# LinjianMa/pairwise-perturbation

Hardware: AMD Instinct MI355X
Metric: ALS sweeps/sec (exact dimension-tree sweep, CP order-4 s=200 R=10) (higher is better)
Workload: dtype f32

## Files before the change

### include/ppals.h

```cpp
#ifndef PPALS_H
#define PPALS_H
#include <stdint.h>
#ifdef __cplusplus
extern "C" {
#endif

#define PPALS_F32 0
#define PPALS_F64 1

#define PPALS_OK 0
#define PPALS_ERR_NO_DEVICE (-1)
#define PPALS_ERR_HIP (-2)
#define PPALS_ERR_ARG (-3)
#define PPALS_ERR_COMM (-4)
#define PPALS_ERR_UNSUPPORTED (-5)
#define PPALS_MAX_ORDER 8
#define PPALS_UNIQUE_ID_BYTES 128

typedef struct ppals_ctx ppals_ctx;
typedef struct ppals_tensor ppals_tensor;
typedef struct ppals_cp ppals_cp;
typedef struct ppals_tucker ppals_tucker;

const char *ppals_last_error(void);
const char *ppals_version(void);

int ppals_preload_eigensolver(void);

int ppals_ctx_create(ppals_ctx **out, int device);
void ppals_ctx_destroy(ppals_ctx *ctx);
int ppals_get_unique_id(void *out128);
int ppals_ctx_init_comm(ppals_ctx *ctx, int rank, int nranks, const void *unique_id128);
int ppals_ctx_rank(const ppals_ctx *ctx);
int ppals_ctx_nranks(const ppals_ctx *ctx);
int ppals_ctx_sync(ppals_ctx *ctx);
int ppals_profile_enable(ppals_ctx *ctx, int level);
int ppals_profile_read(ppals_ctx *ctx, int which, int64_t *launches, double *total_ms,
                       double *algo_bytes);
int ppals_profile_reset(ppals_ctx *ctx);

int ppals_tensor_create(ppals_ctx *ctx, int order, const int64_t *global_lens, int dtype,
                        ppals_tensor **out);
void ppals_tensor_destroy(ppals_tensor *t);
int ppals_tensor_local_rows(const ppals_tensor *t, int64_t *lo, int64_t *n);
int ppals_tensor_fill_cp(ppals_tensor *t, int R, const double *Wtrue_flat);
int ppals_tensor_fill_uniform(ppals_tensor *t, uint64_t seed, double lo, double hi);
int ppals_tensor_fill_laplacian(ppals_tensor *t, int ndigits, int s);
int ppals_tensor_fill_collinear(ppals_tensor *t, int R, double col_min, double col_max,
                                double ratio_noise, uint64_t seed);
int ppals_collinear_factors(int order, const int64_t *lens, int R, double col_min, double col_max,
                            uint64_t seed, double *Wflat);
int ppals_tensor_upload(ppals_tensor *t, const double *host_full);
int ppals_tensor_download(ppals_tensor *t, double *host_full);

#define PPALS_F16 2
#define PPALS_BF16 3
int ppals_tensor_import_device(ppals_tensor *t, const void *src, int src_dtype, const int64_t *box_lo,
                               const int64_t *box_len, const int64_t *strides, void *stream);
int ppals_tensor_export_device(ppals_tensor *t, void *dst, int dst_dtype, const int64_t *box_lo,
                               const int64_t *box_len, const int64_t *strides, void *stream);
int ppals_tensor_check_device_view(ppals_tensor *t, int direction, const void *ptr, int dtype,
                                   const int64_t *box_lo, const int64_t *box_len,
                                   const int64_t *strides);
int ppals_tensor_norm(ppals_tensor *t, double *out);
void ppals_fill_uniform_host(double *out, int64_t n, uint64_t seed, uint64_t offset, double lo,
                             double hi);

int ppals_tree_node(ppals_cp *s, const char *key, double *out, int64_t *n);
int ppals_mttkrp(ppals_cp *s, int mode, double *M);
int ppals_pp_operator(ppals_cp *s, const char *contracted, double *out, int64_t *n);
int ppals_cp_residual(ppals_cp *s, double *out);
int ppals_cp_gram_system(ppals_cp *s, int mode, double lambda, double *S, double *Sinv);

int ppals_cp_create(ppals_ctx *ctx, ppals_tensor *V, int R, ppals_cp **out);
void ppals_cp_destroy(ppals_cp *s);
int ppals_cp_set_factors(ppals_cp *s, const double *Wflat, const double *gradWflat );
int ppals_cp_get_factors(ppals_cp *s, double *Wflat, double *gradWflat );
#define PPALS_SCHEDULE_DT 0
#define PPALS_SCHEDULE_MSDT 1
int ppals_cp_set_schedule(ppals_cp *s, int schedule);
int ppals_cp_get_schedule(const ppals_cp *s);
int ppals_cp_placement_report(const ppals_cp *s, char *buf, int cap);
int ppals_cp_pp_build_stats(ppals_cp *s, int mode, int64_t *builds, double *seconds);
int ppals_cp_sweeps_dt(ppals_cp *s, int n, double lambda);
int ppals_cp_gradnorm(ppals_cp *s, double *out);

typedef struct {
  double tol;
  double timelimit;
  int maxiter;
  double lambda;
  int resprint;
  int bench;
  double tol_init;
  double ratio_step;
  const char *csv_path;
  int csv_append;
  int verbose;
  double update_percentage;
} ppals_cp_opts;

int ppals_cp_dt(ppals_cp *s, const ppals_cp_opts *o, int *iters);
int ppals_cp_pp(ppals_cp *s, const ppals_cp_opts *o, int *iters);
int ppals_cp_pp_partupdate(ppals_cp *s, const ppals_cp_opts *o, int *iters);

#define PPALS_OPT_SIMPLE 0
#define PPALS_OPT_DT 1
#define PPALS_OPT_MSDT 2
int ppals_cpd_als(ppals_cp *s, int optimizer, const ppals_cp_opts *o, double *sweeps, int *iters);
#define PPALS_OPT_DT_LR 3
#define PPALS_OPT_MSDT_LR 4
int ppals_cpd_als_lr(ppals_cp *s, int optimizer, int update_rank, int randomsvd,
                     const ppals_cp_opts *o, double *sweeps, int *iters);

int ppals_tucker_create(ppals_ctx *ctx, ppals_tensor *V, const int *ranks, ppals_tucker **out);
void ppals_tucker_destroy(ppals_tucker *s);
int ppals_tucker_set_factors(ppals_tucker *s, const double *Wflat);
int ppals_tucker_set_core(ppals_tucker *s, const double *core);
int ppals_tucker_get_factors(ppals_tucker *s, double *Wflat, double *core);
int ppals_tucker_hosvd(ppals_tucker *s);
int ppals_tucker_ttmc(ppals_tucker *s, int skip, double *Y, int64_t *n);
int ppals_tucker_sweeps_dt(ppals_tucker *s, int n);
int ppals_tucker_dt(ppals_tucker *s, const ppals_cp_opts *o, int *iters);
int ppals_tucker_pp(ppals_tucker *s, const ppals_cp_opts *o, int *iters);

#define PPALS_MODEL 0
#define PPALS_RESIDUAL 1
int ppals_cp_export_model_device(ppals_cp *s, int what, void *dst, int dst_dtype, const int64_t *box_lo,
                                 const int64_t *box_len, const int64_t *strides, void *stream);
int ppals_tucker_export_model_device(ppals_tucker *s, int what, void *dst, int dst_dtype,
                                     const int64_t *box_lo, const int64_t *box_len,
                                     const int64_t *strides, void *stream);

#ifdef __cplusplus
}
#endif
#endif
```

### pairwise-perturbation_amd/csrc/engine.cpp

```cpp
#include "engine.h"
#include "run_report.h"

#include <algorithm>
#include <cmath>
#include <cstdio>
#include <cstdlib>
#include <cstring>
#include <fstream>
#include <iostream>
#include <stdexcept>

namespace ppals {

int tensor_create(Ops &ops, Comm &comm, int order, const int64_t *glens, int dtype,
                  TensorDesc *out, std::string *err) {
  if (order < 2 || order > MAX_ORDER) {
    *err = "tensor order must be in [2, 8]";
    return -1;
  }
  if (!ops.supports_storage(dtype))
    throw Unsupported(dtype == BF16 ? "ppals: this back end cannot store a bf16 tensor"
                                    : "ppals: this back end cannot store this tensor type");
  TensorDesc t;
  t.order = order;
// ... 132 lines not shown
        if (ok) break;
      }
    }
    W += s * R;
  }
  for (int i = 0; i < R; i++) {
    const double lambda_ = 0.2 + 0.6 / R * (i + 1);
    for (int64_t e = 0; e < lens[0]; e++) Wflat[e + lens[0] * i] *= lambda_;
  }
}

void tensor_fill_collinear(Ops &ops, Comm &comm, const TensorDesc &V, int R, double col_min,
                           double col_max, double ratio_noise, uint64_t seed) {
  size_t tot = 0;
  for (int i = 0; i < V.order; i++) tot += (size_t)V.glens[i] * R;
  std::vector<double> W(tot);
  collinear_factors(V.glens, V.order, R, col_min, col_max, seed, W.data());
  tensor_fill_cp(ops, V, R, W.data());
  const double vnorm = tensor_norm(ops, comm, V);
  double *d = (double *)ops.alloc(sizeof(double));
  const uint64_t nseed = seed + 0x5eedull;
  ops.uniform_sumsq(V.llens[0], V.glens[0], V.row0, rest_of(V), nseed, -1.0, 1.0, d);
  if (comm.size() > 1) comm.allreduce_sum(d, 1);
  double nsq = 0;
  ops.d2h(&nsq, d, sizeof(double));
  ops.free(d);
  const double alpha = ratio_noise * vnorm / std::sqrt(nsq);
  ops.add_uniform_noise(V.data, V.dtype, V.llens[0], V.glens[0], V.row0, rest_of(V), nseed, -1.0,
                        1.0, alpha);
  ops.sync();
}

double tensor_norm(Ops &ops, Comm &comm, const TensorDesc &V) {
  int64_t M, K;
  split_sizes(V, &M, &K);
  double *d = (double *)ops.alloc(sizeof(double));
  ops.residual_sq(V.data, V.dtype, M, K, nullptr, nullptr, 0, d);
  if (comm.size() > 1) comm.allreduce_sum(d, 1);
  double h = 0;
  ops.d2h(&h, d, sizeof(double));
  ops.free(d);
  return std::sqrt(h);
}

CpEngine::CpEngine(Ops &ops, Comm &comm, const TensorDesc &V, int R)
    : ops_(ops), comm_(comm), V_(V), N_(V.order), R_(R), P_(comm.size()), rank_(comm.rank()) {
  dist_ = P_ > 1 || (force_comm_path() && !comm.is_self());
  if (R <= 0) throw std::runtime_error("ppals: rank must be positive");
  residual_form_ = residual_form_env();
  W_.resize(N_);
  gradW_.resize(N_);
  Wprev_.assign(N_, nullptr);
  Winit_.assign(N_, nullptr);
  dW_.assign(N_, nullptr);
  dM_.assign(N_, nullptr);
  Mm_.assign(N_, nullptr);
  for (int i = 0; i < N_; i++) {
    size_t n = (size_t)V_.glens[i] * R_ * sizeof(double);
    W_[i] = (double *)ops_.alloc(n);
    gradW_[i] = (double *)ops_.alloc(n);
    ops_.zero(W_[i], n);
    ops_.zero(gradW_[i], n);
    maxs_ = std::max(maxs_, V_.glens[i]);
    maxblk_ = std::max(maxblk_, block_rows(V_.glens[i], P_));
  }
  G_ = (double *)ops_.alloc(sizeof(double) * N_ * R_ * R_);
  S_ = (double *)ops_.alloc(sizeof(double) * R_ * R_);
  Sinv_ = (double *)ops_.alloc(sizeof(double) * R_ * R_);
  gradsq_ = (double *)ops_.alloc(sizeof(double) * MAX_ORDER);
  scal_ = (double *)ops_.alloc(sizeof(double) * 4 * MAX_ORDER);
  ops_.zero(gradsq_, sizeof(double) * MAX_ORDER);
  if (dist_) {
    size_t n = sizeof(double) * (size_t)maxblk_ * P_ * R_;
    sendbuf_ = (double *)ops_.alloc(n);
    recvbuf_ = (double *)ops_.alloc(sizeof(double) * (size_t)maxblk_ * R_);
    gatherbuf_ = (double *)ops_.alloc(n);
    ops_.zero(sendbuf_, n);
    ops_.zero(gatherbuf_, n);
  }
  if (const char *e = std::getenv("PPALS_COMM_SMALL_BYTES")) small_msg_bytes_ = std::atoll(e);
  if (const char *e = std::getenv("PPALS_TEST_BLOCKED_UPDATE")) test_blocks_ = std::atoi(e);
  if (N_ < 3) schedule_ = 0;
  if (const char *e = std::getenv("PPALS_PLACE_TUNE")) ms_tune_enabled_ = std::atoi(e) != 0;
  if (N_ >= 3) {
    ms_set_roots(ms_choose_roots());
    ms_scales_ = (double *)ops_.alloc(sizeof(double) * 32);
  }
  if (V_.generation) tensor_gen_ = *V_.generation;
  {
    Layout nat;
    nat.ptr = V_.data;
    for (int m = 0; m < N_; m++) nat.order.push_back(m);
    lay_.push_back(nat);
  }
  size_t xmax = 0;
  const bool place = schedule_ == 1 && N_ >= 3 && ms_tune_enabled_ && ms_X_slack() > 0;
  if (place) {
    for (int r = 0; r < N_; r++) {
      if (ms_set_excluded(r, ms_k_, ms_excl_)) continue;
      xmax = std::max(xmax, ms_X_bytes(r, ms_k_));
    }
    const size_t avail = ops_.mem_available();
    const double tensor_bytes = (double)V_.nloc * dtype_size(V_.dtype);
    if (avail == (size_t)-1 || (double)avail > 2.0 * tensor_bytes + 6.0 * (double)(xmax + ms_X_slack()) + 8e9)
      ms_X_alt_ = ops_.try_alloc(xmax + ms_X_slack());
  }
  ensure_transposed();
  if (place) {
    ms_X_base_ = big_alloc(xmax + ms_X_slack());
    ms_X_cap_ = xmax + ms_X_slack();
  }
  for (int i = 0; i < MAX_ORDER; i++) grad_replicated_[i] = !dist_;
  build_tree(0, N_ - 1, -1);
  leaf_.assign(N_, -1);
  for (size_t k = 0; k < nodes_.size(); k++)
    if (nodes_[k].lo == nodes_[k].hi) leaf_[nodes_[k].lo] = (int)k;
}

void CpEngine::set_schedule(int schedule) {
  if (schedule != 0 && schedule != 1) throw std::runtime_error("ppals: unknown sweep schedule");
  schedule_ = (N_ < 3) ? 0 : schedule;
  for (auto &n : nodes_) n.valid = false;
  ms_invalidate();
}

CpEngine::~CpEngine() {
  try {
    ops_.sync();
  } catch (...) {
  }
  for (auto p : W_) ops_.free(p);
  for (auto p : gradW_) ops_.free(p);
  for (auto p : Wprev_) ops_.free(p);
  for (auto p : Winit_) ops_.free(p);
  for (auto p : dW_) ops_.free(p);
  for (auto p : dM_) ops_.free(p);
  for (auto p : Mm_) ops_.free(p);
  for (auto &n : nodes_) ops_.free(n.buf);
  lr_release();
  pp_clear();
  for (auto &kv : pp_pool_) ops_.free(kv.second.buf);
  ops_.free(pp_norms_);
  ops_.free(G_);
  ops_.free(S_);
  ops_.free(Sinv_);
  ops_.free(gradsq_);
  ops_.free(scal_);
  ops_.free(sendbuf_);
  ops_.free(recvbuf_);
  ops_.free(gatherbuf_);
  ops_.free(test_blkbuf_);
  ops_.free(Mbuf_);
  ops_.free(Qbuf_);
  ops_.free(xq_);
  ops_.free(xp_);
  ops_.free(Pbuf_);
  for (auto &l : lay_)
    if (l.owned) ops_.free(l.ptr);
  for (auto &ex : ms_place_)
    if (ex.timer >= 0) ops_.timer_read(ex.timer);
  ops_.free(ms_X_base_);
  ops_.free(ms_X_alt_);
  ops_.free(ms_scales_);
  for (auto &n : ms_nodes_) {
    ops_.free(n.t.buf);
    for (auto &t : n.tmp) ops_.free(t.buf);
// ... 44 lines not shown
        l.q = q;
        l.blk = b;
        l.ld = ld;
        return;
      }
    }
  };
  auto bytes_of = [&](const Layout &l) {
    return l.q ? (size_t)l.ld * (size_t)(V_.nloc / l.blk) * esz : (size_t)V_.nloc * esz;
  };
  const int mid = (N_ - 1) / 2;
  Layout t;
  for (int m = mid + 1; m < N_; m++) t.order.push_back(m);
  for (int m = 0; m <= mid; m++) t.order.push_back(m);
  choose_pad(t, std::min(N_ - 2, N_ - 1 - mid));
  int64_t min_ext = ext(0);
  for (int m = 1; m < N_; m++) min_ext = std::min(min_ext, ext(m));
  const size_t xbytes_max = (size_t)(V_.nloc / std::max<int64_t>(1, min_ext)) * R_ * esz;
  const size_t reserve = 3 * xbytes_max + ms_X_slack() + ((size_t)1 << 30);
  auto fits = [&](size_t bytes) {
    const size_t avail = ops_.mem_available();
    return avail == (size_t)-1 || avail >= bytes + reserve;
  };
  if (!fits(bytes_of(t))) return;
  t.ptr = ops_.try_alloc(bytes_of(t));
  if (!t.ptr) return;
  t.owned = true;
  t.bytes = bytes_of(t);
  fill_layout(t);
  lay_.push_back(t);
  vt_state_ = 1;
  Layout a;
  for (int m = 0; m < N_; m++) a.order.push_back(m);
  choose_pad(a, N_ - 2);
  if (a.q > 0 && fits(bytes_of(a))) {
    a.ptr = ops_.try_alloc(bytes_of(a));
    if (a.ptr) {
      a.owned = true;
      a.bytes = bytes_of(a);
      fill_layout(a);
      lay_.push_back(a);
    }
  }
}

bool CpEngine::plan_scan(int first, int k, bool natural_only, ScanPlan &plan) {
  auto in_set = [&](int m) { return ((m - first + N_) % N_) < k; };
  const int64_t line = 128 / (int64_t)dtype_size(V_.dtype);
  const Layout *best = nullptr;
  int best_p0 = 0;
  int64_t best_L = 0;
  bool best_al = false;
  const size_t nlay = natural_only ? 1 : lay_.size();
  for (size_t li = 0; li < nlay; li++) {
    const Layout &l = lay_[li];
    int p0 = -1;
    for (int p = 0; p < N_; p++)
      if (in_set(l.order[p])) {
        p0 = p;
        break;
      }
    int len = 0;
    while (p0 + len < N_ && in_set(l.order[p0 + len])) len++;
    if (len != k || (l.q > 0 && p0 < l.q)) continue;
    int64_t L = 1;
    for (int p = 0; p < p0; p++) L *= ext(l.order[p]);
    const bool al = L >= 256 && (l.q > 0 || L % line == 0);
    if (!best || (al && !best_al) ||
        (al == best_al && (L > best_L || (L == best_L && l.q > 0 && best->q == 0)))) {
      best = &l;
      best_p0 = p0;
      best_L = L;
      best_al = al;
    }
  }
  if (!best) return false;
  plan = ScanPlan();
  plan.lay = best;
  for (int p = 0; p < N_; p++) {
    const int m = best->order[p];
    if (p < best_p0) {
      plan.Lc *= ext(m);
      plan.kept.push_back(m);
    } else if (p < best_p0 + k) {
      plan.J *= ext(m);
      plan.set.push_back(m);
    } else {
      plan.T *= ext(m);
      plan.kept.push_back(m);
    }
  }
  plan.L = plan.Lc;
  if (best->q > 0) {
    plan.L = plan.Lc / best->blk * best->ld;
    plan.pad.ld = best->ld;
    plan.pad.valid = best->blk;
  }
  return true;
}

void CpEngine::check_tensor_generation() {
  if (!V_.generation || *V_.generation == tensor_gen_) return;
  tensor_gen_ = *V_.generation;
  for (const auto &l : lay_)
    if (l.owned) fill_layout(l);
  for (auto &n : nodes_) n.valid = false;
  ms_invalidate();
  pp_clear();
}

FactorRef CpEngine::fref(int m, double *const *W) const {
  FactorRef f;
  f.ptr = W[m] + (m == 0 ? V_.row0 : 0);
  f.rows = ext(m);
  f.ld = V_.glens[m];
  return f;
}
int64_t CpEngine::prod_ext(int lo, int hi) const {
  int64_t p = 1;
  for (int m = lo; m <= hi; m++) p *= ext(m);
  return p;
}

void CpEngine::build_tree(int lo, int hi, int parent) {
  if (hi <= lo) return;
  const int mid = (lo + hi) / 2;
  const int ranges[2][2] = {{lo, mid}, {mid + 1, hi}};
  int idx[2];
  for (int c = 0; c < 2; c++) {
    Node n;
    n.lo = ranges[c][0];
    n.hi = ranges[c][1];
    n.parent = parent;
    n.slo = ranges[1 - c][0];
    n.shi = ranges[1 - c][1];
    n.elems = 0;
    nodes_.push_back(n);
    idx[c] = (int)nodes_.size() - 1;
  }
  build_tree(lo, mid, idx[0]);
  build_tree(mid + 1, hi, idx[1]);
}
int CpEngine::find_node(int lo, int hi) const {
  for (size_t k = 0; k < nodes_.size(); k++)
    if (nodes_[k].lo == lo && nodes_[k].hi == hi) return (int)k;
  return -1;
}

void CpEngine::compute_node(int idx) {
  check_tensor_generation();
  Node &n = nodes_[idx];
  if (n.valid) return;
  n.elems = prod_ext(n.lo, n.hi);
  if (!n.buf) n.buf = (double *)ops_.alloc(sizeof(double) * (size_t)n.elems * R_);
  FactorRef f[MAX_ORDER];
  int nf = 0;
  for (int m = n.slo; m <= n.shi; m++) f[nf++] = fref(m, W_.data());
  const int64_t J = prod_ext(n.slo, n.shi);
  const bool sib_is_suffix = n.slo > n.hi;
  if (n.parent < 0) {
    ScanPlan pl;
    if (!plan_scan(n.slo, n.shi - n.slo + 1, false, pl))
      throw std::runtime_error("ppals: internal error (tree node not adjacent)");
    if (pl.Lc == 1 && !sib_is_suffix) {
      ops_.scan_contract(V_.data, V_.dtype, 1, J, n.elems, f, nf, R_, n.buf, F64, 1, n.elems);
    } else {
// ... 204 lines not shown
  }
}

bool CpEngine::ms_set_excluded(int first, int k, unsigned excl) const {
  for (int q = 0; q < k; q++)
    if ((excl >> ((first + q) % N_)) & 1u) return true;
  return false;
}

int CpEngine::ms_next_root(int i, int k, unsigned excl) const {
  int first = (i - k + N_) % N_, guard = 0;
  while (ms_set_excluded(first, k, excl) && guard++ < N_) first = (first - 1 + N_) % N_;
  if (ms_set_excluded(first, k, excl) || ((i - first + N_) % N_) < k) return -1;
  return first;
}

double CpEngine::ms_schedule_cost(int k, unsigned excl) const {
  int root = -1;
  double cost = 0;
  const int sweeps = 2 * N_;
  for (int u = 0; u < (sweeps + 2) * N_; u++) {
    const int i = u % N_;
    if (root < 0 || ((i - root + N_) % N_) < k) {
      root = ms_next_root(i, k, excl);
      if (root < 0) return 1e300;
      if (u >= 2 * N_) {
        double J = 1;
        for (int q = 0; q < k; q++) J *= (double)ext((root + q) % N_);
        cost += 1.0 + 4.5 * (double)R_ / J;
      }
    }
  }
  return cost / sweeps;
}

int CpEngine::ms_choose_roots() {
  const unsigned mandatory = (dist_ && N_ > 2) ? 1u : 0u;
  const int kcap = dist_ ? std::max(1, (N_ - 1) / 2) : N_;
  int kfix = 0;
  if (const char *e = std::getenv("PPALS_MSDT_ROOTS")) {
    const int k = std::atoi(e);
    if (k >= 1 && k <= N_ - 2) kfix = std::min(k, kcap);
  }
  unsigned small = 0;
  for (int m = 0; m < N_; m++)
    if ((double)R_ >= 0.05 * (double)ext(m)) small |= 1u << m;
  int best = 1;
  unsigned best_excl = mandatory;
  double best_cost = 1e300;
  for (int k = 1; k <= std::max(1, N_ / 2) && k <= N_ - 2 && k <= kcap; k++) {
    if (kfix && k != kfix) continue;
    for (unsigned sub = small;; sub = (sub - 1) & small) {
      const unsigned excl = sub | mandatory;
      const double cost = ms_schedule_cost(k, excl);
      const bool tie = cost <= best_cost * (1.0 + 1e-9) && cost >= best_cost * (1.0 - 1e-9);
      if (cost < best_cost * (1.0 - 1e-9) ||
          (tie && k == best && __builtin_popcount(excl) < __builtin_popcount(best_excl))) {
        best_cost = cost;
        best = k;
        best_excl = excl;
      }
      if (sub == 0) break;
    }
  }
  if (best_cost >= 1e299) {
    best = 1;
    best_excl = mandatory;
  }
  ms_excl_ = best_excl;
  return best;
}

void CpEngine::ms_set_roots(int k) {
  for (auto &n : ms_nodes_) {
    ops_.free(n.t.buf);
    for (auto &t : n.tmp) ops_.free(t.buf);
  }
  ms_nodes_.clear();
  ms_k_ = k;
  ms_build_tree(0, N_ - k - 1, -1);
  ms_leaf_.assign(N_ - k, -1);
  for (size_t q = 0; q < ms_nodes_.size(); q++)
    if (ms_nodes_[q].lo == ms_nodes_[q].hi) ms_leaf_[ms_nodes_[q].lo] = (int)q;
  if (ms_nodes_.size() + 1 > 32) throw std::runtime_error("ppals: tensor order too large");
  ms_X_.slot = 0;
  for (size_t q = 0; q < ms_nodes_.size(); q++) ms_nodes_[q].t.slot = (int)q + 1;
  ms_invalidate();
}

double CpEngine::place_min_bytes() {
  const char *e = std::getenv("PPALS_PLACE_MIN_MB");
  return e ? std::atof(e) * 1048576.0 : 1.5e9;
}

size_t CpEngine::ms_X_slack() const {
  const double bytes = (double)V_.nloc * dtype_size(V_.dtype);
  return bytes >= place_min_bytes() ? ((size_t)64 << 20) + 4096 : 0;
}

void CpEngine::ms_place_collect(PlaceExplore &ex) {
  if (ex.timer < 0) return;
  const double t = ops_.timer_read(ex.timer);
  ex.timer = -1;
  if (t <= 0 || ex.timer_cand < 0 || ex.timer_cand >= (int)ex.cands.size()) return;
  PlaceCand &c = ex.cands[ex.timer_cand];
  c.best = std::min(c.best, t);
  c.samples++;
  ex.worst = std::max(ex.worst, t);
}

int CpEngine::ms_place_pick(PlaceExplore &ex) {
  ms_place_collect(ex);
  if (ex.phase == 0) {
    int n = 0, best0 = -1;
    double lo = 1e300, hi = 0;
    for (size_t q = 0; q < ex.cands.size(); q++)
      if (ex.cands[q].samples > 0) {
        n++;
        lo = std::min(lo, ex.cands[q].best);
        hi = std::max(hi, ex.cands[q].best);
        if (ex.cands[q].blk == 0 && (best0 < 0 || ex.cands[q].best < ex.cands[best0].best)) best0 = (int)q;
      }
    if (n >= kPlaceGateSamples && best0 >= 0 && hi < lo * (1.0 + kPlaceGateSpread)) {
      ex.chosen = best0;
      ex.gated = true;
      ex.phase = 2;
      ms_place_release_unchosen();
      return -1;
    }
  }
  if (ex.phase == 0 && ex.next >= ex.cands.size()) {
    std::vector<int> idx(ex.cands.size());
    for (size_t q = 0; q < idx.size(); q++) idx[q] = (int)q;
    std::stable_sort(idx.begin(), idx.end(),
                     [&](int a, int b) { return ex.cands[a].best < ex.cands[b].best; });
    const size_t nfin = std::min<size_t>(3, idx.size());
    for (size_t q = 0; q < nfin; q++)
      for (int kind = 0; kind < 2; kind++) {
        PlaceCand c;
        c.blk = ex.cands[idx[q]].blk;
        c.off = ex.cands[idx[q]].off;
        c.nt = kind;
        ex.cands.push_back(c);
      }
    ex.phase = 1;
  }
  if (ex.phase == 1 && ex.next >= ex.cands.size()) {
    int best = -1;
    for (size_t q = 0; q < ex.cands.size(); q++)
      if (ex.cands[q].samples > 0 && (best < 0 || ex.cands[q].best < ex.cands[best].best * 0.995))
        best = (int)q;
    ex.chosen = best;
    ex.phase = 2;
    ms_place_release_unchosen();
  }
  return ex.phase < 2 ? (int)ex.next++ : -1;
}

void CpEngine::ms_place_release_unchosen() {
  if (!ms_X_alt_) return;
  bool use[2] = {false, false};
  for (const auto &ex : ms_place_) {
    if (ex.phase == 0 || ex.phase == 1) return;
    if (ex.phase == 2) use[ex.chosen >= 0 ? ex.cands[ex.chosen].blk : 0] = true;
  }
  if (use[0] && use[1]) return;
  ops_.sync();
  if (!use[1]) {
    ops_.free(ms_X_alt_);
  } else {
    ops_.free(ms_X_base_);
    ms_X_base_ = ms_X_alt_;
    for (auto &ex : ms_place_)
      for (auto &c : ex.cands) c.blk = 0;
  }
  ms_X_alt_ = nullptr;
}

size_t CpEngine::ms_X_bytes(int first, int k) const {
  int64_t J = 1;
  for (int q = 0; q < k; q++) J *= ext((first + q) % N_);
  return (size_t)(V_.nloc / J) * R_ * dtype_size(work_dt(V_.dtype));
}

void *CpEngine::big_alloc(size_t bytes) {
  for (;;) {
    void *p = ops_.try_alloc(bytes);
    if (p) return p;
    if (ms_X_alt_ && !(ms_X_.valid && (char *)ms_X_.buf >= (char *)ms_X_alt_ &&
                       (char *)ms_X_.buf < (char *)ms_X_alt_ + ms_X_cap_)) {
      ops_.sync();
      for (auto &ex : ms_place_) {
        if (ex.timer >= 0) {
          ops_.timer_read(ex.timer);
          ex.timer = -1;
        }
        for (auto &c : ex.cands) c.blk = 0;
      }
      ops_.free(ms_X_alt_);
      ms_X_alt_ = nullptr;
      continue;
    }
    if (lay_.size() > 1 && lay_.back().owned) {
      ops_.sync();
      ops_.free(lay_.back().ptr);
      lay_.pop_back();
      if (lay_.size() == 1) vt_state_ = -1;
      for (auto &n : nodes_) n.valid = false;
      continue;
    }
    return ops_.alloc(bytes);
  }
}

void CpEngine::ms_start_step(int first) {
  const int k = ms_k_;
  ms_root_ = first;
  ms_order_.clear();
  for (int q = k; q < N_; q++) ms_order_.push_back((first + q) % N_);
  for (auto &n : ms_nodes_) n.t.valid = false;
  const size_t xbytes = ms_X_bytes(first, k);
  const size_t slack = ms_tune_enabled_ ? ms_X_slack() : 0;
  if (!ms_X_override_ && ms_X_cap_ < xbytes + slack) {
    for (auto &ex : ms_place_) {
      if (ex.timer >= 0) ops_.timer_read(ex.timer);
      ex = PlaceExplore();
    }
    ops_.free(ms_X_base_);
    ops_.free(ms_X_alt_);
    ms_X_base_ = ms_X_alt_ = nullptr;
    ms_X_cap_ = 0;
    ms_X_base_ = big_alloc(xbytes + slack);
    ms_X_cap_ = xbytes + slack;
  }
  ScanPlan pl;
  if (!plan_scan(first, k, false, pl)) {
    if (k == 1) throw std::runtime_error("ppals: internal error (single root not adjacent)");
    ms_set_roots(1);
    int r = (first + k - 1) % N_, guard = 0;
    while (((ms_excl_ >> r) & 1u) && guard++ < N_) r = (r - 1 + N_) % N_;
    ms_start_step(r);
    return;
  }
  const void *src = pl.lay->ptr;
  const int64_t L = pl.Lc, J = pl.J, T = pl.T;
  ms_X_.modes = pl.kept;
  std::vector<FactorRef> f;
  unsigned mask = 0;
  for (int m : pl.set) {
    f.push_back(fref(m, W_.data()));
    mask |= 1u << m;
  }
  ms_X_.dt = work_dt(V_.dtype);
  ms_X_.contracted = mask;
  if ((size_t)L * T * R_ * dtype_size(ms_X_.dt) != xbytes)
    throw std::runtime_error("ppals: internal error (first-level intermediate size)");
  auto launch_scan = [&](int blk, int64_t off, int nt) {
    ms_X_.buf = ms_X_override_ ? (char *)ms_X_override_
                               : (char *)(blk == 1 && ms_X_alt_ ? ms_X_alt_ : ms_X_base_) + off;
    ops_.scan_store_mode(nt);
    ops_.scan_contract(src, V_.dtype, pl.L, J, T, f.data(), (int)f.size(), R_, ms_X_.buf, ms_X_.dt,
                       L, L * T, pl.pad);
    ops_.scan_store_mode(-1);
  };
  PlaceExplore &ex = ms_place_[first];
  if (slack > 0 && !ms_X_override_ && ex.phase < 0) {
    static const int64_t cand_small[] = {0, 1, 2, 3, 4, 5, 6, 8, 12, 16, 24, 32, 48, 64};
    static const int64_t cand_large[] = {0, 3, 5, 12, 16, 24, 48, 64};
    const double bytes = (double)L * J * T * dtype_size(V_.dtype);
    ex.phase = 3;
    ex.layout = (int)(pl.lay - lay_.data());
    if (bytes >= place_min_bytes() && R_ <= 32 && (double)xbytes >= 0.01 * bytes) {
      const bool large = bytes >= 2e10;
      const int64_t *mb = large ? cand_large : cand_small;
      for (int ci = 0; ci < (large ? 8 : 14); ci++) {
        if ((size_t)(mb[ci] << 20) > slack) break;
        PlaceCand c;
        c.off = mb[ci] << 20;
        ex.cands.push_back(c);
      }
      static const int64_t cand_alt[] = {0, 4, 16, 64};
      for (int ci = 0; ms_X_alt_ && ci < 4; ci++) {
        if ((size_t)(cand_alt[ci] << 20) > slack) break;
        PlaceCand c;
        c.blk = 1;
        c.off = cand_alt[ci] << 20;
        ex.cands.push_back(c);
      }
      ex.phase = 0;
    }
  }
  const int cand = (slack > 0 && !ms_X_override_ && ex.phase >= 0 && ex.phase < 2) ? ms_place_pick(ex) : -1;
  if (cand >= 0) {
    ex.visits++;
    ex.timer_cand = cand;
    ex.timer = ops_.timer_begin();
    launch_scan(ex.cands[cand].blk, ex.cands[cand].off, ex.cands[cand].nt);
    if (ex.timer >= 0) ops_.timer_end(ex.timer);
  } else if (ex.phase == 2 && ex.chosen >= 0 && slack > 0 && !ms_X_override_) {
    launch_scan(ex.cands[ex.chosen].blk, ex.cands[ex.chosen].off, ex.cands[ex.chosen].nt);
  } else {
    launch_scan(0, 0, -1);
  }
  ms_X_.pending = false;
  ms_X_.valid = true;
  if (const char *tr = std::getenv("PPALS_TRACE_STEPS")) {
    if (FILE *f = std::fopen(tr, "a")) {
      const int li = (int)(pl.lay - lay_.data());
      std::fprintf(f, "rank=%d root=%d k=%d layout=%s%s L=%lld J=%lld T=%lld\n", rank_, first, k,
                   li == 1 ? "VT" : "V", pl.lay->q > 0 ? "pad" : "", (long long)L, (long long)J,
                   (long long)T);
      std::fclose(f);
    }
  }
}

void CpEngine::ms_mode_update(int i, double lambda, bool last_of_sweep) {
  check_tensor_generation();
  if (ms_root_ < 0 || ((i - ms_root_ + N_) % N_) < ms_k_) {
    const int first = ms_next_root(i, ms_k_, ms_excl_);
    if (first < 0) throw std::runtime_error("ppals: no root set without the excluded modes");
    ms_start_step(first);
  }
  int pos = -1;
  for (size_t q = 0; q < ms_order_.size(); q++)
    if (ms_order_[q] == i) pos = (int)q;
  const int leaf = ms_leaf_[pos];
  ops_.arm_gram_system(G_, N_, i, R_, lambda, S_, Sinv_);
  ms_compute(leaf);
  ms_norm_fused_ = false;
  if (last_of_sweep && (!dist_ || (i != 0 && (int64_t)sizeof(double) * V_.glens[i] * R_ <= small_msg_bytes_))) {
    int64_t rows[MAX_ORDER];
    for (int q = 0; q < N_; q++) rows[q] = V_.glens[q];
    if (ops_.arm_normalize(W_.data(), rows, N_, R_, G_, i, nullptr)) {
      unsigned masks[32] = {0}, fresh = 0;
      const unsigned active = ms_collect_scales(masks, &fresh, leaf);
      ms_norm_fused_ = ops_.arm_normalize(W_.data(), rows, N_, R_, G_, i, nullptr, ms_scales_, masks, active, fresh);
    }
  }
  mode_update(i, (const double *)ms_nodes_[leaf].t.buf, ext(i), lambda, false, 1.0);
  ms_nodes_[leaf].t.valid = false;
}

void CpEngine::ms_contract(const RTensor &src, int mode, RTensor &dst, const double *in_scale) {
  int64_t L = 1, T = 1;
  bool before = true;
  dst.modes.clear();
  for (int m : src.modes) {
    if (m == mode) {
      before = false;
      continue;
    }
    (before ? L : T) *= ext(m);
    dst.modes.push_back(m);
  }
  dst.dt = F64;
  dst.contracted = src.contracted | (1u << mode);
  ms_reserve(dst, sizeof(double) * (size_t)L * T * R_);
  FactorRef f = fref(mode, W_.data());
  ops_.mttv(src.buf, src.dt, L, ext(mode), T, &f, 1, R_, (double *)dst.buf, L * T, 0, in_scale);
}

void CpEngine::ms_compute(int idx) {
  MsNode &n = ms_nodes_[idx];
  if (n.t.valid) return;
  const RTensor *src;
  if (n.parent < 0) {
    src = &ms_X_;
  } else {
    ms_compute(n.parent);
    src = &ms_nodes_[n.parent].t;
  }
  std::vector<int> sib;
  for (int pos = n.slo; pos <= n.shi; pos++) sib.push_back(ms_order_[pos]);
  auto storage_pos = [&](int mode) {
    for (size_t k = 0; k < src->modes.size(); k++)
      if (src->modes[k] == mode) return (int)k;
    return -1;
  };
  std::sort(sib.begin(), sib.end(), [&](int a, int b) { return storage_pos(a) > storage_pos(b); });
  if (n.tmp.size() + 1 < sib.size()) n.tmp.resize(sib.size() - 1);
  const RTensor *cur = src;
  for (size_t k = 0; k < sib.size(); k++) {
    RTensor &dst = (k + 1 == sib.size()) ? n.t : n.tmp[k];
    ms_contract(*cur, sib[k], dst, k == 0 ? ms_scale_of(*src) : nullptr);
    cur = &dst;
  }
  if (sib.empty()) throw std::runtime_error("ppals: empty sibling set in the multi-sweep tree");
  n.t.pending = false;
  n.t.valid = true;
}

void CpEngine::sweep_msdt(double lambda) {
  for (int i = 0; i < N_; i++) ms_mode_update(i, lambda, i == N_ - 1);
  if (!ms_norm_fused_) normalize();
  ms_norm_fused_ = false;
  grad_from_sweep_ = true;
}

void CpEngine::sweep_dt(double lambda) {
  if (schedule_ == 1) {
    sweep_msdt(lambda);
    return;
  }
  for (auto &n : nodes_) n.valid = false;
  bool norm_fused = false;
  for (int i = 0; i < N_; i++) {
    compute_node(leaf_[i]);
    const Node &lf = nodes_[leaf_[i]];
    if (i == N_ - 1 && !dist_) {
      int64_t rows[MAX_ORDER];
      for (int q = 0; q < N_; q++) rows[q] = V_.glens[q];
      norm_fused = ops_.arm_normalize(W_.data(), rows, N_, R_, G_, i, nullptr);
    }
    mode_update(i, lf.buf, ext(i), lambda, false, 1.0);
  }
  if (!norm_fused) normalize();
  grad_from_sweep_ = true;
}

void CpEngine::update_modes(int first, int count, double lambda) {
  for (int k = 0; k < count; k++) {
    const int i = (first + k) % N_;
    if (schedule_ == 1) {
      ms_mode_update(i, lambda);
    } else {
      if (i == 0 || k == 0)
        for (auto &n : nodes_) n.valid = false;
      compute_node(leaf_[i]);
      mode_update(i, nodes_[leaf_[i]].buf, ext(i), lambda, false, 1.0);
    }
  }
  grad_from_sweep_ = true;
}

void CpEngine::lr_release() {
  for (int m = 0; m < MAX_ORDER; m++) {
    ops_.free(lr_cache_[m]);
    lr_cache_[m] = nullptr;
    lr_have_[m] = false;
  }
  ops_.free(lr_X_);
  ops_.free(lr_Us_);
  ops_.free(lr_G2_);
  ops_.free(lr_small_);
  ops_.free(lr_T_);
  lr_X_ = lr_Us_ = lr_G2_ = lr_small_ = lr_T_ = nullptr;
  lr_T_cap_ = 0;
}

void CpEngine::lr_step_begin(int left, bool reuse, int r) {
  check_tensor_generation();
  if (ms_k_ != 1) ms_set_roots(1);
  if (!lr_cache_[left]) lr_cache_[left] = big_alloc(ms_X_bytes(left, 1));
  if (reuse && lr_have_[left]) {
    ScanPlan pl;
    if (!plan_scan(left, 1, false, pl)) throw std::runtime_error("ppals: internal error (LR scan plan)");
    const int64_t n = pl.Lc * pl.T;
    if (lr_T_cap_ < sizeof(double) * (size_t)n * r) {
      ops_.free(lr_T_);
      lr_T_ = (double *)ops_.alloc(sizeof(double) * (size_t)n * r);
      lr_T_cap_ = sizeof(double) * (size_t)n * r;
    }
    FactorRef f;
    f.ptr = lr_Us_ + (left == 0 ? V_.row0 : 0);
    f.rows = ext(left);
    f.ld = V_.glens[left];
    ops_.scan_contract(pl.lay->ptr, V_.dtype, pl.L, ext(left), pl.T, &f, 1, r, lr_T_, F64, pl.Lc, n,
                       pl.pad);
    ops_.lowrank_accumulate(lr_cache_[left], work_dt(V_.dtype), n, R_, lr_T_, r, lr_small_);
    ms_X_ = lr_desc_[left];
    ms_X_.buf = lr_cache_[left];
    ms_X_.valid = true;
    ms_X_.pending = false;
    ms_root_ = left;
    ms_order_.clear();
    for (int q = 1; q < N_; q++) ms_order_.push_back((left + q) % N_);
    for (auto &nd : ms_nodes_) nd.t.valid = false;
  } else {
    ms_X_override_ = lr_cache_[left];
    ms_start_step(left);
    ms_X_override_ = nullptr;
    lr_desc_[left] = ms_X_;
    lr_have_[left] = true;
  }
}

static void host_qr_mgs2(int n, int k, double *A) {
  for (int j = 0; j < k; j++) {
    double *aj = A + (size_t)n * j;
    for (int pass = 0; pass < 2; pass++)
      for (int p = 0; p < j; p++) {
        const double *ap = A + (size_t)n * p;
        double d = 0;
        for (int i = 0; i < n; i++) d += ap[i] * aj[i];
        for (int i = 0; i < n; i++) aj[i] -= d * ap[i];
      }
    double nn = 0;
    for (int i = 0; i < n; i++) nn += aj[i] * aj[i];
    nn = std::sqrt(nn);
    for (int i = 0; i < n; i++) aj[i] = nn > 0 ? aj[i] / nn : 0.0;
  }
}
static void host_jacobi_eig(int n, double *A, double *ev, double *V) {
  for (int i = 0; i < n; i++)
    for (int j = 0; j < n; j++) V[i + (size_t)n * j] = i == j ? 1.0 : 0.0;
  for (int sweep = 0; sweep < 60; sweep++) {
    double off = 0, diag = 0;
    for (int i = 0; i < n; i++)
      for (int j = 0; j < n; j++) (i == j ? diag : off) += A[i + (size_t)n * j] * A[i + (size_t)n * j];
    if (off <= 1e-30 * (diag + 1e-300)) break;
    for (int p = 0; p < n - 1; p++)
      for (int q = p + 1; q < n; q++) {
        const double apq = A[p + (size_t)n * q];
        if (apq == 0.0) continue;
        const double theta = (A[q + (size_t)n * q] - A[p + (size_t)n * p]) / (2.0 * apq);
        const double t = (theta >= 0 ? 1.0 : -1.0) / (std::fabs(theta) + std::sqrt(theta * theta + 1.0));
        const double c = 1.0 / std::sqrt(t * t + 1.0), sn = t * c;
        for (int k = 0; k < n; k++) {
          const double akp = A[k + (size_t)n * p], akq = A[k + (size_t)n * q];
          A[k + (size_t)n * p] = c * akp - sn * akq;
          A[k + (size_t)n * q] = sn * akp + c * akq;
        }
        for (int k = 0; k < n; k++) {
          const double apk = A[p + (size_t)n * k], aqk = A[q + (size_t)n * k];
          A[p + (size_t)n * k] = c * apk - sn * aqk;
          A[q + (size_t)n * k] = sn * apk + c * aqk;
        }
        for (int k = 0; k < n; k++) {
          const double vkp = V[k + (size_t)n * p], vkq = V[k + (size_t)n * q];
          V[k + (size_t)n * p] = c * vkp - sn * vkq;
          V[k + (size_t)n * q] = sn * vkp + c * vkq;
        }
      }
  }
  std::vector<int> idx(n);
  for (int i = 0; i < n; i++) idx[i] = i;
  std::sort(idx.begin(), idx.end(), [&](int a, int b) { return A[a + (size_t)n * a] > A[b + (size_t)n * b]; });
  std::vector<double> Vs((size_t)n * n);
  for (int k = 0; k < n; k++) {
    ev[k] = A[idx[k] + (size_t)n * idx[k]];
    for (int i = 0; i < n; i++) Vs[i + (size_t)n * k] = V[i + (size_t)n * idx[k]];
  }
  std::copy(Vs.begin(), Vs.end(), V);
}
static const uint64_t LR_RANDOM_SEED = 0x52414e44535644ull;

void CpEngine::lr_mode_update(int i, double lambda, int r, const double *base) {
  int pos = -1;
  for (size_t q = 0; q < ms_order_.size(); q++)
    if (ms_order_[q] == i) pos = (int)q;
  if (pos < 0) throw std::runtime_error("ppals: internal error (LR update of the root mode)");
  const int leaf = ms_leaf_[pos];
  ms_compute(leaf);
  const double *M = (const double *)ms_nodes_[leaf].t.buf;
  const int64_t s = V_.glens[i];
  if (r <= 0) {
    mode_update(i, M, ext(i), lambda, false, 1.0);
    ms_nodes_[leaf].t.valid = false;
    return;
  }
// ... 871 lines not shown
```

### pairwise-perturbation_amd/csrc/engine.h

```cpp
#pragma once
#include <cstdint>
#include <cstdlib>
#include <map>
#include <string>
#include <vector>

#include "ops.h"

namespace ppals {

struct TensorDesc {
  int order = 0;
  int64_t glens[MAX_ORDER];
  int64_t llens[MAX_ORDER];
  int64_t row0 = 0;
  int dtype = F32;
  void *data = nullptr;
  int64_t nloc = 0;
  const uint64_t *generation = nullptr;
};

inline int64_t block_rows(int64_t s, int P) { return (s + P - 1) / P; }
inline bool force_comm_path() {
  const char *v = getenv("PPALS_FORCE_COMM");
  return v && atoi(v) != 0;
}

enum ResidualForm { RESIDUAL_FUSED = 0, RESIDUAL_TWO_PASS = 1 };
int residual_form_env();
struct ModelExportCall {
  const ViewArgs *a;
  const TensorDesc *V;
  void *dst;
  bool residual;
  int form;
  bool exported = false;
  void *stream;
};
void model_export_run(Ops &ops, ModelExportCall &c, const ModelPlan &mp, const double *Q, const double *P,
                      int K);

int tensor_create(Ops &ops, Comm &comm, int order, const int64_t *glens, int dtype,
                  TensorDesc *out, std::string *err);
void tensor_fill_cp(Ops &ops, const TensorDesc &V, int R, const double *Wtrue_flat);
void tensor_fill_uniform(Ops &ops, const TensorDesc &V, uint64_t seed, double lo, double hi);
void tensor_upload(Ops &ops, const TensorDesc &V, const double *host_full);
void tensor_download(Ops &ops, const TensorDesc &V, double *host_full);
void tensor_fill_laplacian(Ops &ops, const TensorDesc &V, int ndigits, int s);
void collinear_factors(const int64_t *lens, int N, int R, double col_min, double col_max,
                       uint64_t seed, double *Wflat);
void tensor_fill_collinear(Ops &ops, Comm &comm, const TensorDesc &V, int R, double col_min,
                           double col_max, double ratio_noise, uint64_t seed);
double tensor_norm(Ops &ops, Comm &comm, const TensorDesc &V);

struct CpOpts {
  double tol = 0, timelimit = 5e3;
  int maxiter = 0;
  double lambda = 0;
  int resprint = 10;
  int bench = 0;
  double tol_init = 1e-2, ratio_step = 1.0;
  double update_percentage = 1.0;
  int update_rank = 0;
  int randomsvd = 0;
  std::string csv_path;
  bool csv_append = false;
  bool verbose = false;
};

class RunReport;
struct ModeNorms;

class CpEngine {
 public:
  CpEngine(Ops &ops, Comm &comm, const TensorDesc &V, int R);
  ~CpEngine();

  void set_factors(const double *Wflat, const double *gradWflat);
  void set_schedule(int schedule);
  int schedule() const { return schedule_; }
  std::string placement_report() const;
  void pp_build_stats(int mode, int64_t *builds, double *seconds) {
    if (builds) *builds = pp_builds_;
    if (seconds) *seconds = pp_build_s_;
    if (mode != 0) {
      pp_builds_ = 0;
      pp_build_s_ = 0;
      pp_build_timed_ = mode > 0;
    }
  }
  void get_factors(double *Wflat, double *gradWflat);

  void sweep_dt(double lambda);
  double gradnorm();
  double residual();
  void export_model(const ViewArgs &a, void *dst, bool residual, void *stream);
  const TensorDesc &tensor() const { return V_; }

  int64_t tree_node(const std::string &key, double *out_host);
  void mttkrp(int mode, double *M_host);
  int64_t pp_operator(const std::string &contracted, double *out_host);
  void gram_system(int mode, double lambda, double *S_host, double *Sinv_host);

  int run_dt(const CpOpts &o, int *iters);
  int run_pp(const CpOpts &o, int *iters);
  int run_pp_partupdate(const CpOpts &o, int *iters);
  int run_class(int kind, const CpOpts &o, double *sweeps, int *iters);
  void update_modes(int first, int count, double lambda);


  int order() const { return N_; }
  int rank_r() const { return R_; }

 private:
  struct Node {
    int lo, hi;
    int parent = -1;
    int slo, shi;
    double *buf = nullptr;
    int64_t elems = 0;
    bool valid = false;
  };
  struct PPOp {
    void *buf = nullptr;
    int dt = F64;
    int64_t elems = 0;
    std::vector<int> modes;
    bool owned = true;
    const double *scale = nullptr;
  };
  struct PPBuf {
    void *buf = nullptr;
    size_t cap = 0;
  };
  std::map<std::string, PPBuf> pp_pool_;
  void *pp_buffer(const std::string &seq, size_t bytes);
  bool pp_norms_live_ = false;
  double *pp_norms_ = nullptr;

  struct RTensor {
    void *buf = nullptr;
    size_t cap = 0;
    int dt = F64;
    std::vector<int> modes;
    unsigned contracted = 0;
    int slot = -1;
    bool pending = false;
    bool valid = false;
  };
  struct MsNode {
    int lo, hi, parent, slo, shi;
    RTensor t;
    std::vector<RTensor> tmp;
  };
  void ms_build_tree(int lo, int hi, int parent);
  void ms_start_step(int root);
  void ms_compute(int idx);
  void ms_reserve(RTensor &t, size_t bytes);
  void ms_contract(const RTensor &src, int mode, RTensor &dst, const double *in_scale);
  void sweep_msdt(double lambda);
  void ms_invalidate() { ms_root_ = -1; }
  int schedule_ = 1;
  int ms_root_ = -1;
  int ms_k_ = 1;
  int test_blocks_ = 0;
  double *test_blkbuf_ = nullptr;
  unsigned ms_excl_ = 0;
  bool ms_set_excluded(int first, int k, unsigned excl) const;
  int ms_next_root(int i, int k, unsigned excl) const;
  double ms_schedule_cost(int k, unsigned excl) const;
  int ms_choose_roots();
  void ms_set_roots(int k);
  void ms_mode_update(int i, double lambda, bool last_of_sweep = false);
  bool ms_norm_fused_ = false;
  unsigned ms_collect_scales(unsigned *masks, unsigned *fresh, int skip_node);
  RTensor ms_X_;
  struct PlaceCand {
    int blk = 0;
    int64_t off = 0;
    int nt = -1;
    double best = 1e300;
    int samples = 0;
  };
  struct PlaceExplore {
    int phase = -1;
    size_t next = 0;
    int timer = -1;
    int timer_cand = -1;
    int chosen = -1;
    int layout = 0;
    double worst = 0;
    int visits = 0;
    bool gated = false;
    std::vector<PlaceCand> cands;
  };
  static constexpr int kPlaceGateSamples = 8;
  static constexpr double kPlaceGateSpread = 0.04;
  PlaceExplore ms_place_[MAX_ORDER];
  void ms_place_collect(PlaceExplore &ex);
  int ms_place_pick(PlaceExplore &ex);
  void *ms_X_base_ = nullptr;
  void *ms_X_alt_ = nullptr;
  void ms_place_release_unchosen();
  size_t ms_X_cap_ = 0;
  int64_t pp_builds_ = 0;
  double pp_build_s_ = 0;
  bool pp_build_timed_ = false;
  bool ms_tune_enabled_ = true;
  size_t ms_X_slack() const;
  static double place_min_bytes();
  size_t ms_X_bytes(int first, int k) const;
  void *big_alloc(size_t bytes);
  std::vector<MsNode> ms_nodes_;
  void lr_step_begin(int left, bool reuse, int r);
  void lr_mode_update(int i, double lambda, int r, const double *base);
  void lr_release();
  void *lr_cache_[MAX_ORDER] = {nullptr};
  bool lr_have_[MAX_ORDER] = {false};
  bool lr_random_ = false;
  uint64_t lr_random_calls_ = 0;
  RTensor lr_desc_[MAX_ORDER];
  void *ms_X_override_ = nullptr;
  double *lr_X_ = nullptr, *lr_Us_ = nullptr, *lr_G2_ = nullptr, *lr_small_ = nullptr;
  double *lr_T_ = nullptr;
  size_t lr_T_cap_ = 0;


  std::vector<int> ms_order_;
  std::vector<int> ms_leaf_;
  double *ms_scales_ = nullptr;
  const double *ms_scale_of(const RTensor &t) const { return t.pending ? ms_scales_ + t.slot : nullptr; }

  int64_t ext(int m) const { return m == 0 ? V_.llens[0] : V_.glens[m]; }
  FactorRef fref(int m, double *const *W) const;
  int64_t prod_ext(int lo, int hi) const;
  void build_tree(int lo, int hi, int parent);
  int find_node(int lo, int hi) const;
  void compute_node(int idx);
  void refresh_grams();
  void mode_update(int i, const double *M, int64_t ldm, double lambda, bool pp, double ratio);
  void normalize();
  const PPOp &pp_get(const std::string &seq);
  int pp_last_mode(const std::string &seq) const;
  std::string pp_parent(const std::string &seq) const;
  void pp_contract_pair(const PPOp &T, int cmode, const FactorRef &f, double *out, int64_t out_rows);
  bool pp_fast_ = true;
  bool pp_no_borrow_ = false;
  void pp_clear();
  void pp_build_all();
  void sweep_pp(double lambda, double ratio);
  double allreduce_scalar(double x);
  bool agree(bool local);
  ModeNorms read_norms(bool dt_phase);
  bool print_block(RunReport &rep, const CpOpts &o, int iter, int pp_flag, double &projnorm,
                   bool bench);
  void dt_sub(RunReport &rep, const CpOpts &o, double &projnorm, int &iter);
  void pp_restart();
  void pp_sub(RunReport &rep, const CpOpts &o, double &projnorm, int &iter);
  void pp_partupdate_sub(RunReport &rep, const CpOpts &o, double &projnorm, int &iter);
  int run_pp_common(const CpOpts &o, int *iters, bool partupdate);

  Ops &ops_;
  Comm &comm_;
  TensorDesc V_;
  int N_, R_, P_, rank_;
  bool dist_ = false;
  std::vector<double *> W_, gradW_, Wprev_, Winit_, dW_, dM_, Mm_;
  double *G_ = nullptr;
  double *S_ = nullptr, *Sinv_ = nullptr;
  double *gradsq_ = nullptr;
  double *scal_ = nullptr;
  double *sendbuf_ = nullptr, *recvbuf_ = nullptr, *gatherbuf_ = nullptr;
  double *Mbuf_ = nullptr;
  double *Qbuf_ = nullptr, *Pbuf_ = nullptr;
  double *xq_ = nullptr, *xp_ = nullptr;
  int64_t xq_cap_ = 0, xp_cap_ = 0;
  int residual_form_ = RESIDUAL_FUSED;
  struct Layout {
    void *ptr = nullptr;
    std::vector<int> order;
    int q = 0;
    int64_t blk = 0, ld = 0;
    bool owned = false;
    size_t bytes = 0;
  };
  std::vector<Layout> lay_;
  int vt_state_ = 0;
  uint64_t tensor_gen_ = 0;
  void ensure_transposed();
  void fill_layout(const Layout &l);
  struct ScanPlan {
    const Layout *lay = nullptr;
    int64_t L = 1, Lc = 1, J = 1, T = 1;
    RowPad pad;
    std::vector<int> set, kept;
  };
  bool plan_scan(int first, int k, bool natural_only, ScanPlan &plan);
  void check_tensor_generation();
  int64_t small_msg_bytes_ = 1 << 20;
  bool grad_replicated_[MAX_ORDER];
  int64_t maxs_ = 0, maxblk_ = 0;
  std::vector<Node> nodes_;
  std::vector<int> leaf_;
  std::map<std::string, PPOp> pp_;
  bool grad_from_sweep_ = false;
  double init_gradnorm_ = 0;
};

}
```

### pairwise-perturbation_amd/csrc/hip_ops.hip

```cpp
#include <dlfcn.h>
#include <hip/hip_runtime.h>
#include <chrono>

#include <algorithm>
#include <cstdio>
#include <cstdlib>
#include <stdexcept>
#include <string>
#include <map>
#include <type_traits>
#include <vector>

#include "hip_ops.h"
#include "roctx_ranges.h"
#include "preload_policy.h"
#include "kernels_scan.hip.h"
#include "kernels_small.hip.h"
#include "kernels_eig.hip.h"
#include "kernels_io.hip.h"
#include "kernels_model.hip.h"
#include "kernels_bf16.hip.h"

namespace ppals {
#define HIP_CHECK(expr)                                                                       \
// ... 28 lines not shown

template <auto V, auto... Vs, typename T, typename F>
static inline void dispatch(T v, F &&f) {
  if constexpr (sizeof...(Vs) == 0)
    f(std::integral_constant<decltype(V), V>());
  else if (v == V)
    f(std::integral_constant<decltype(V), V>());
  else
    dispatch<Vs...>(v, f);
}

struct EigLibs {
  void *blas = nullptr, *solver = nullptr;
};
static bool g_hip_runtime_up = false;
static EigLibs &eig_libs() {
  static EigLibs l;
  if (l.blas && l.solver) return l;
  switch (late_preload_policy(false, g_hip_runtime_up, getenv("PPALS_STRICT_PRELOAD"))) {
    case kPreloadRefuse: throw Unsupported(late_preload_message());
    case kPreloadWarn: fprintf(stderr, "%s\n", late_preload_message()); fflush(stderr); break;
    default: break;
  }
  l.blas = dlopen("librocblas.so.5", RTLD_NOW | RTLD_GLOBAL);
  if (!l.blas) l.blas = dlopen("librocblas.so", RTLD_NOW | RTLD_GLOBAL);
  l.solver = dlopen("librocsolver.so.0", RTLD_NOW | RTLD_GLOBAL);
  if (!l.solver) l.solver = dlopen("librocsolver.so", RTLD_NOW | RTLD_GLOBAL);
  if (!l.blas || !l.solver)
    throw std::runtime_error(std::string("ppals: cannot load rocSOLVER: ") + dlerror());
  return l;
}

class HipOps : public Ops {
 public:
  explicit HipOps(int device) {
    int ndev = 0;
    hipError_t e = hipGetDeviceCount(&ndev);
    if (e != hipSuccess || ndev <= 0)
      throw std::runtime_error(
          "ppals: no HIP device available (the engine has no CPU fallback; hipGetDeviceCount: " +
          std::string(e == hipSuccess ? "0 devices" : hipGetErrorString(e)) + ")");
    if (device < 0 || device >= ndev)
      throw std::runtime_error("ppals: device index out of range");
    dev_ = device;
    g_hip_runtime_up = true;
    HIP_CHECK(hipSetDevice(dev_));
    HIP_CHECK(hipStreamCreateWithFlags(&st_, hipStreamNonBlocking));
    hipDeviceProp_t prop;
    HIP_CHECK(hipGetDeviceProperties(&prop, dev_));
    ncu_ = prop.multiProcessorCount;
    HIP_CHECK(hipFuncSetAttribute((const void *)k_gram_system,
                                  hipFuncAttributeMaxDynamicSharedMemorySize, 96 * 1024));
    HIP_CHECK(hipFuncSetAttribute((const void *)k_cp_update,
                                  hipFuncAttributeMaxDynamicSharedMemorySize, 96 * 1024));
    HIP_CHECK(hipFuncSetAttribute((const void *)k_top_eig_small,
                                  hipFuncAttributeMaxDynamicSharedMemorySize, 152 * 1024));
    HIP_CHECK(hipFuncSetAttribute((const void *)k_cp_mode_update<false, false>,
                                  hipFuncAttributeMaxDynamicSharedMemorySize, 152 * 1024));
    HIP_CHECK(hipFuncSetAttribute((const void *)k_cp_mode_update<true, true>,
                                  hipFuncAttributeMaxDynamicSharedMemorySize, 152 * 1024));
    if (const char *v = getenv("PPALS_FORCE_JACOBI")) force_jacobi_ = atoi(v);
    if (const char *v = getenv("PPALS_EIG_FAST")) {
      eig_fast_ = atoi(v);
      eig_cold_ = eig_fast_ != 2;
    }
    if (const char *v = getenv("PPALS_EIG_DEBUG")) eig_debug_ = atoi(v);
    if (const char *v = getenv("PPALS_EIG_SIGMA_SCALE")) eig_sigma_scale_ = atof(v);
    if (const char *v = getenv("PPALS_FORCE_EIGINV")) force_eiginv_ = atoi(v);
    HIP_CHECK(hipFuncSetAttribute((const void *)k_chol_rinv,
                                  hipFuncAttributeMaxDynamicSharedMemorySize, 72 * 1024));
    HIP_CHECK(hipFuncSetAttribute((const void *)k_chol_m,
                                  hipFuncAttributeMaxDynamicSharedMemorySize, 152 * 1024));
    HIP_CHECK(hipFuncSetAttribute((const void *)k_rr_apply,
                                  hipFuncAttributeMaxDynamicSharedMemorySize, 152 * 1024));
    if (const char *v = getenv("PPALS_SYM_LDS_MIN")) sym_lds_min_ = std::max(32, atoi(v));
    if (const char *v = getenv("PPALS_EIG_DEFER")) {
      eig_defer_ok_ = atoi(v);
      handover_ok_ = eig_defer_ok_ != 2;
    }
    if (const char *v = getenv("PPALS_EIG_DEFER_FAIL")) eig_defer_fail_ = atoi(v);
    if (const char *v = getenv("PPALS_SCAN_TAIL")) scan_tail_on_ = atoi(v) != 0;
    if (const char *v = getenv("PPALS_SCAN_WIDE")) wide_enabled_ = atoi(v) != 0;
    if (const char *v = getenv("PPALS_COLD_SUBSPACE_FROM")) cold_subspace_from_ = std::max(65, atoi(v));
    if (const char *v = getenv("PPALS_PERSIST_MULT")) persist_mult_ = std::max(1, atoi(v));
    HIP_CHECK(hipFuncSetAttribute((const void *)k_rmult_chol,
                                  hipFuncAttributeMaxDynamicSharedMemorySize, 152 * 1024));
    HIP_CHECK(hipFuncSetAttribute((const void *)k_jacobi_onesided,
                                  hipFuncAttributeMaxDynamicSharedMemorySize, 152 * 1024));
    HIP_CHECK(hipFuncSetAttribute((const void *)k_rr_small,
                                  hipFuncAttributeMaxDynamicSharedMemorySize, 152 * 1024));
    HIP_CHECK(hipFuncSetAttribute((const void *)k_gram_system_lds,
                                  hipFuncAttributeMaxDynamicSharedMemorySize, 152 * 1024));
    HIP_CHECK(hipFuncSetAttribute((const void *)k_gram_system_mfma,
                                  hipFuncAttributeMaxDynamicSharedMemorySize, 152 * 1024));
    if (const char *v = getenv("PPALS_GJ_SCALAR")) gj_scalar_ = atoi(v);
  }
  ~HipOps() override {
    hipSetDevice(dev_);
    hipStreamSynchronize(st_);
    if (st2_) hipStreamSynchronize(st2_);
    for (auto &ev : events_) {
      hipEventDestroy(ev.a);
      hipEventDestroy(ev.b);
    }
    for (auto &t : timers_) {
      hipEventDestroy(t.a);
      hipEventDestroy(t.b);
    }
    if (ws_mttv_) hipFree(ws_mttv_);
    if (ws_pack_) hipFree(ws_pack_);
    if (ws_mv_) hipFree(ws_mv_);
    if (ws_slab_) hipFree(ws_slab_);
    if (ws_krp_) hipFree(ws_krp_);
    if (ws_part_) hipFree(ws_part_);
    if (ws_small_) hipFree(ws_small_);
    if (ws_big_) hipFree(ws_big_);
    if (ws_big2_) hipFree(ws_big2_);
    if (ws_eig_) hipFree(ws_eig_);
    if (ws_orth_) hipFree(ws_orth_);
    if (ws_pow_) hipFree(ws_pow_);
    if (ws_cold_) hipFree(ws_cold_);
    if (ws_cold2_) hipFree(ws_cold2_);
    if (ws_cholm_) hipFree(ws_cholm_);
    if (ws_gsfb_) hipFree(ws_gsfb_);
    if (ws_jac_) hipFree(ws_jac_);
    if (eig_host_) hipHostFree(eig_host_);
    if (ws_part2_) hipFree(ws_part2_);
    for (auto &kv : eig_state_) {
      if (kv.second.Q) hipFree(kv.second.Q);
      if (kv.second.Qn) hipFree(kv.second.Qn);
      free_lazy(kv.second);
    }
    for (auto &kv : eig_small_)
      if (kv.second.Q) hipFree(kv.second.Q);
    if (st2_) hipStreamDestroy(st2_);
    if (handover_) hipFree(handover_);
    if (io_ev_in_) hipEventDestroy(io_ev_in_);
    if (io_ev_out_) hipEventDestroy(io_ev_out_);
    hipStreamDestroy(st_);
  }

  void *alloc(size_t bytes) override {
    void *p = nullptr;
    HIP_CHECK(hipSetDevice(dev_));
    HIP_CHECK(hipMalloc(&p, bytes ? bytes : 8));
    return p;
  }
  void free(void *p) override {
    if (p) {
      hipStreamSynchronize(st_);
      hipFree(p);
    }
  }
  void h2d(void *dst, const void *src, size_t bytes) override {
    HIP_CHECK(hipMemcpyAsync(dst, src, bytes, hipMemcpyHostToDevice, st_));
    HIP_CHECK(hipStreamSynchronize(st_));
  }
  void d2h(void *dst, const void *src, size_t bytes) override {
    HIP_CHECK(hipMemcpyAsync(dst, src, bytes, hipMemcpyDeviceToHost, st_));
    HIP_CHECK(hipStreamSynchronize(st_));
  }
  void d2d(void *dst, const void *src, size_t bytes) override {
    HIP_CHECK(hipMemcpyAsync(dst, src, bytes, hipMemcpyDeviceToDevice, st_));
  }
  void zero(void *p, size_t bytes) override { HIP_CHECK(hipMemsetAsync(p, 0, bytes, st_)); }
  void sync() override { HIP_CHECK(hipStreamSynchronize(st_)); }
  void *stream() override { return (void *)st_; }
  void bind() override { HIP_CHECK(hipSetDevice(dev_)); }
  bool supports_storage(int dt) override { return dt == F32 || dt == F64 || dt == BF16; }

  void fill_uniform(void *V, int dt, int64_t l0, int64_t g0, int64_t row0, int64_t rest,
                    uint64_t seed, double lo, double hi) override {
    int64_t n = l0 * rest;
    int g = grid_for(n, 256, 16384);
    if (dt == F32)
      hipLaunchKernelGGL(k_fill_uniform<float>, dim3(g), dim3(256), 0, st_, (float *)V, l0, g0,
                         row0, rest, seed, lo, hi);
    else if (dt == BF16)
      hipLaunchKernelGGL(k_fill_uniform<bf16s>, dim3(g), dim3(256), 0, st_, (bf16s *)V, l0, g0,
                         row0, rest, seed, lo, hi);
    else
      hipLaunchKernelGGL(k_fill_uniform<double>, dim3(g), dim3(256), 0, st_, (double *)V, l0, g0,
                         row0, rest, seed, lo, hi);
    HIP_CHECK(hipGetLastError());
  }

  void fill_laplacian(void *V, int dt, int64_t l0, int64_t g0, int64_t row0, int64_t rest,
                      int ndigits, int s) override {
    int g = grid_for(l0 * rest, 256, 16384);
    if (dt == F32)
      hipLaunchKernelGGL(k_fill_laplacian<float>, dim3(g), dim3(256), 0, st_, (float *)V, l0, g0,
                         row0, rest, ndigits, s);
    else if (dt == BF16)
      hipLaunchKernelGGL(k_fill_laplacian<bf16s>, dim3(g), dim3(256), 0, st_, (bf16s *)V, l0, g0,
                         row0, rest, ndigits, s);
// ... 413 lines not shown
  }

  void *try_alloc(size_t bytes) override {
    void *p = nullptr;
    hipSetDevice(dev_);
    if (hipMalloc(&p, bytes ? bytes : 8) != hipSuccess) {
      (void)hipGetLastError();
      return nullptr;
    }
    return p;
  }
  void scan_store_mode(int mode) override { scan_nt_mode_ = mode; }
  int scan_nt_mode_ = -1;
  size_t mem_available() override {
    size_t fr = 0, tot = 0;
    hipSetDevice(dev_);
    if (hipMemGetInfo(&fr, &tot) != hipSuccess) {
      (void)hipGetLastError();
      return (size_t)-1;
    }
    return fr;
  }
  void unpack_shards(const void *stage, int dt, int64_t s0, int64_t rest, int64_t blk, int P,
                     int64_t chunk_bytes, void *full) override {
    const int g = grid_for(s0 * rest, 256, 16384);
    if (dt == F32)
      hipLaunchKernelGGL(k_unpack_shards<float>, dim3(g), dim3(256), 0, st_, (const char *)stage,
                         s0, rest, blk, P, chunk_bytes, (float *)full);
    else if (dt == BF16)
      hipLaunchKernelGGL(k_unpack_shards<bf16s>, dim3(g), dim3(256), 0, st_, (const char *)stage,
                         s0, rest, blk, P, chunk_bytes, (bf16s *)full);
    else
      hipLaunchKernelGGL(k_unpack_shards<double>, dim3(g), dim3(256), 0, st_, (const char *)stage,
                         s0, rest, blk, P, chunk_bytes, (double *)full);
    HIP_CHECK(hipGetLastError());
  }
  void transpose2d(const void *src, int dt, int64_t rows, int64_t cols, void *dst) override {
    transpose_batched(src, dt, rows, cols, 1, dst);
  }
  void transpose_batched(const void *src, int dt, int64_t rows, int64_t cols, int64_t batch,
                         void *dst) override {
    const int64_t nb = ((rows + 63) / 64) * ((cols + 63) / 64);
    if (nb > 0x7fffffff) throw std::runtime_error("ppals: transpose grid too large");
    const size_t step = (size_t)rows * cols * dtype_size(dt);
    for (int64_t b0 = 0; b0 < batch; b0 += 65535) {
      const unsigned nby = (unsigned)std::min<int64_t>(65535, batch - b0);
      const char *s = (const char *)src + b0 * step;
      char *d = (char *)dst + b0 * step;
      if (dt == F32)
        hipLaunchKernelGGL(k_transpose<float>, dim3((unsigned)nb, nby), dim3(256), 0, st_,
                           (const float *)s, rows, cols, (float *)d);
      else if (dt == BF16)
        hipLaunchKernelGGL(k_transpose<bf16s>, dim3((unsigned)nb, nby), dim3(256), 0, st_,
                           (const bf16s *)s, rows, cols, (bf16s *)d);
      else
        hipLaunchKernelGGL(k_transpose<double>, dim3((unsigned)nb, nby), dim3(256), 0, st_,
                           (const double *)s, rows, cols, (double *)d);
    }
    HIP_CHECK(hipGetLastError());
  }

  static KrpArgs krp_args(const FactorRef *f, int nf, int64_t *J) {
    KrpArgs a;
    int64_t j = 1;
    if (nf > MAX_ORDER) throw std::runtime_error("ppals: too many Khatri-Rao factors");
    for (int i = 0; i < nf; i++) {
      a.ptr[i] = f[i].ptr;
      a.rows[i] = f[i].rows;
      a.ld[i] = f[i].ld;
      j *= f[i].rows;
    }
    a.nf = nf;
    *J = j;
    return a;
  }
  void krp(double *out, const FactorRef *f, int nf, int col0, int ncols) override {
    int64_t J;
    KrpArgs a = krp_args(f, nf, &J);
    hipLaunchKernelGGL(k_krp, dim3(grid_for(J * ncols, 256)), dim3(256), 0, st_, out, a, J, col0,
                       ncols);
    HIP_CHECK(hipGetLastError());
  }

  template <typename TV>
  void scan_t(const TV *V, int64_t L, int64_t J, int64_t T, const FactorRef *f, int nf, int R,
              double *out, int64_t out_tstride, int64_t out_rstride, int out32, RowPad pad) {
    constexpr int VEC = ScanTraits<TV>::VEC;
    int64_t Jc;
    KrpArgs a = krp_args(f, nf, &Jc);
    if (Jc != J) throw std::runtime_error("ppals: scan_contract factor extents do not match J");
    if (pad.ld && (L % pad.ld || pad.ld % VEC || pad.valid > pad.ld || pad.valid <= 0 || L == 1))
      throw std::runtime_error("ppals: scan_contract padded rows inconsistent");
    const bool aligned_base = (((uintptr_t)V) & 15) == 0;
    const bool wide_ok = sizeof(TV) == 4 && wide_enabled_ && L > 1 && aligned_base && (L % 4 == 0) &&
                         L >= 4 && (double)L * J * T >= 1.0e6 && 16.0 * (double)L * 4.0 < 2.0e9 &&
                         ((double)J / 16.0 + 1.0) * 8.0 * 1024.0 < 2.0e9;
    int col_step = 64;
    for (int col0 = 0; col0 < R; col0 += col_step) {
      if (wide_ok && R - col0 > 64) {
        col_step = std::min(128, R - col0);
        if constexpr (sizeof(TV) == 4)
          scan_wide((const float *)V, L, J, T, a, col0, col_step, out, out_tstride, out_rstride, out32, pad);
        continue;
      }
      col_step = 64;
      const int ncols = std::min(64, R - col0);
      const int NT = ncols <= 16 ? 1 : (ncols <= 32 ? 2 : (ncols <= 48 ? 3 : 4));
      const int64_t nblk64 = (J + 4 * VEC - 1) / (4 * VEC);
      if (nblk64 > 0x7fffffff) throw std::runtime_error("ppals: contraction extent too large");
      const int nblk = (int)nblk64;
      const size_t pack_bytes = (size_t)nblk * NT * 4 * 16 * VEC * sizeof(TV);
      TV *P = (TV *)ensure(ws_pack_, ws_pack_sz_, pack_bytes);
      const bool prefix = (L == 1);
      hipLaunchKernelGGL(k_krp_pack<TV>, dim3(grid_for((int64_t)nblk * NT * 64 * VEC, 256)),
                         dim3(256), 0, st_, P, nblk, NT, prefix ? 1 : 0, a, J, col0, ncols);
      HIP_CHECK(hipGetLastError());
      double *o = out32 ? (double *)((float *)out + (int64_t)col0 * out_rstride)
                        : out + (int64_t)col0 * out_rstride;
      const double bytes = (double)L * (double)J * (double)T * sizeof(TV) +
                           (double)L * (double)T * ncols * (out32 ? 4.0 : 8.0);
      if (prefix) {
        const int64_t M = J, K = T;
        const bool al = aligned_base && (M % VEC == 0);
        const int64_t ncolgrp = (K + 63) / 64;
        int want = 1;
        const int target = ncu_ * 4;
        if (ncolgrp < target) want = (int)std::min<int64_t>((target + ncolgrp - 1) / ncolgrp,
                                                            std::max(1, nblk / 64));
        const KSplit ks = k_split(nblk, want);
        const int nsplit = ks.nsplit, per = (int)ks.per;
        double *dst = o;
        int dst32 = out32;
        int64_t dst_ks = out_tstride, dst_ns = out_rstride, dst_ss = 0;
        if (nsplit > 1) {
          dst32 = 0;
          dst = (double *)ensure(ws_slab_, ws_slab_sz_, sizeof(double) * nsplit * ncols * K);
          dst_ks = 1;
          dst_ns = K;
          dst_ss = (int64_t)ncols * K;
        }
        dim3 grid((unsigned)ncolgrp, (unsigned)nsplit);
        dim3 grid_il((unsigned)((K + 15) / 16), (unsigned)nsplit);
        prof_begin(0, bytes);
        dispatch<1, 2, 3, 4>(NT, [&](auto nt) {
          if (al && M >= VEC)
            hipLaunchKernelGGL((k_scan_prefix_fast<TV, nt, 12>), grid_il, dim3(256), 0, st_, V, M, K, P, per,
                               nblk, dst, dst_ks, dst_ns, dst_ss, ncols, dst32);
          else
            dispatch<true, false>(al, [&](auto alv) {
              hipLaunchKernelGGL((k_scan_prefix<TV, nt, alv, 4>), grid, dim3(256), 0, st_, V, M, K, P, per,
                                 nblk, dst, dst_ks, dst_ns, dst_ss, ncols, dst32);
            });
        });
        prof_end();
        HIP_CHECK(hipGetLastError());
        slab_combine(nsplit, dst, dst_ss, K, ncols, o, out_tstride, out_rstride, out32);
      } else {
        const int64_t M = L, K = J;
        const bool al = aligned_base && (M % VEC == 0);
        const int64_t n_mtiles64 = (M + 64 * VEC - 1) / (64 * VEC);
        const int n_mtiles = (int)n_mtiles64;
        int want = 1;
        const int target = ncu_ * 8;
        if (T == 1 && n_mtiles < target)
          want = (int)std::min<int64_t>((target + n_mtiles - 1) / n_mtiles,
                                        std::max(1, nblk / 32));
        else if (T > 1 && n_mtiles64 * T < ncu_ && (double)M * T * ncols * nblk / 4 * 8.0 < 64e6)
          want = (int)std::min<int64_t>(((int64_t)ncu_ * 2 + n_mtiles64 * T - 1) / (n_mtiles64 * T),
                                        std::max(1, nblk / 4));
        const KSplit ks = k_split(nblk, want);
        const int nsplit = ks.nsplit, per = (int)ks.per;
        const PassDst d = pass_dst(nsplit, M, T, ncols, o, out32, out_rstride, out_tstride, pad);
        const int64_t nblocks = (int64_t)n_mtiles * nsplit * T;
        if (nblocks > 0x7fffffff) throw std::runtime_error("ppals: scan grid too large");
        dim3 grid((unsigned)nblocks);
        prof_begin(0, bytes);
        const int64_t pgrid = nblocks < (int64_t)ncu_ * persist_mult_ ? (int64_t)ncu_ * std::min(persist_mult_, 6)
                                                                       : (int64_t)ncu_ * persist_mult_;
        dim3 grid_p((unsigned)std::min<int64_t>(nblocks, pgrid));
        bool nts = nt_store(nsplit, (double)M * T * ncols * (d.out32 ? 4.0 : 8.0));
        const bool buf_ok = (16.0 * (double)M * sizeof(TV) < 2.0e9) && (pack_bytes < 2000000000ull);
        const bool takes_buf = al && M >= VEC && buf_ok && (NT == 1 || sizeof(TV) == 8) &&
                               !(sizeof(TV) == 8 && nsplit > 1);
        const bool takes_tail = !takes_buf && al && M >= VEC && T == 1 && nsplit == 1 && NT <= 2 &&
                                d.row_ld == 0 && scan_tail_split<TV>(NT, n_mtiles) >= 0;
        if (takes_tail) nts = false;
        if (takes_tail) {
          const int tail_from = scan_tail_split<TV>(NT, n_mtiles);
          const int64_t strips = ((M + 16 * VEC - 1) / (16 * VEC)) - (int64_t)tail_from * 4;
          dim3 grid_t((unsigned)(tail_from + strips));
          const size_t lds_t = sizeof(double) * 3 * (size_t)(VEC * NT * 4) * 64;
          dispatch<1, 2>(NT, [&](auto nt) {
            hipLaunchKernelGGL((k_scan_suffix_fast<TV, nt, 9>), grid_t, dim3(256), lds_t, st_, V, M, K, M * K, P,
                               n_mtiles, nsplit, per, nblk, d.p, d.nstride, d.split_stride, d.batch_stride, ncols,
                               d.out32, (int64_t)0, (int64_t)0, tail_from);
          });
        } else {
          dispatch<1, 2, 3, 4>(NT, [&](auto nt) {
            if (takes_buf)
              dispatch<5, 1>(nts ? 5 : 1, [&](auto opt) {
                hipLaunchKernelGGL((k_scan_suffix_buf<TV, nt, opt>), grid_p, dim3(256), 0, st_, V, M, K, M * K, P,
                                   n_mtiles, nsplit, per, nblk, d.p, d.nstride, d.split_stride, d.batch_stride,
                                   ncols, d.out32, nblocks, d.row_ld, d.row_valid);
              });
            else if (al && M >= VEC)
              dispatch<5, 1>(nts ? 5 : 1, [&](auto opt) {
                hipLaunchKernelGGL((k_scan_suffix_fast<TV, nt, opt>), grid, dim3(256), 0, st_, V, M, K, M * K, P,
                                   n_mtiles, nsplit, per, nblk, d.p, d.nstride, d.split_stride, d.batch_stride,
                                   ncols, d.out32, d.row_ld, d.row_valid);
              });
            else
              dispatch<true, false>(al, [&](auto alv) {
                hipLaunchKernelGGL((k_scan_suffix<TV, nt, alv>), grid, dim3(256), 0, st_, V, M, K, M * K, P,
                                   n_mtiles, nsplit, per, nblk, d.p, d.nstride, d.split_stride, d.batch_stride,
                                   ncols, d.out32, d.row_ld, d.row_valid);
              });
          });
        }
        prof_end();
        HIP_CHECK(hipGetLastError());
        slab_combine(nsplit, d.p, d.split_stride, M, ncols, o, 1, out_rstride, out32, pad, T, d.batch_stride,
                     out_tstride);
      }
    }
  }
  void scan_wide(const float *V, int64_t L, int64_t J, int64_t T, const KrpArgs &a, int col0, int ncols,
                 double *out, int64_t out_tstride, int64_t out_rstride, int out32, RowPad pad) {
    const int NT = (ncols + 15) / 16;
    const int64_t nblk64 = (J + 15) / 16;
    if (nblk64 > 0x7fffffff) throw std::runtime_error("ppals: contraction extent too large");
    const int nblk = (int)nblk64;
    const size_t pack_bytes = (size_t)nblk * NT * 256 * sizeof(float);
    float *P = (float *)ensure(ws_pack_, ws_pack_sz_, pack_bytes);
    hipLaunchKernelGGL(k_krp_pack<float>, dim3(grid_for((int64_t)nblk * NT * 256, 256)), dim3(256), 0, st_,
                       P, nblk, NT, 0, a, J, col0, ncols);
    HIP_CHECK(hipGetLastError());
    double *o = out32 ? (double *)((float *)out + (int64_t)col0 * out_rstride)
                      : out + (int64_t)col0 * out_rstride;
    const int64_t M = L, K = J;
    const int64_t n_mtiles64 = (M + 63) / 64;
    if (n_mtiles64 * T > 0x7fffffff) throw std::runtime_error("ppals: scan grid too large");
    const int n_mtiles = (int)n_mtiles64;
    const void *kernel = nullptr;
    dispatch<5, 6, 7, 8>(NT, [&](auto nt) { kernel = (const void *)k_scan_wide<nt, 1>; });
    const double slots = (double)ncu_ * occupancy(wide_occ_[NT - 1], kernel, 512, 0, 2);
    const int64_t tiles = n_mtiles64 * T;
    int want = 1;
    if ((double)tiles < 8.0 * slots) {
      double best = -1.0;
      const int ns_max = (int)std::min<int64_t>(24, std::max(1, nblk / 16));
      for (int ns = 1; ns <= ns_max; ns++) {
        const double rounds = (double)tiles * ns / slots;
        const double score = rounds / std::ceil(rounds) - 0.004 * ns;
        if (score > best) {
          best = score;
          want = ns;
        }
      }
    }
    const KSplit ks = k_split(nblk, want);
    const int nsplit = ks.nsplit, per = (int)ks.per;
    const PassDst d = pass_dst(nsplit, M, T, ncols, o, out32, out_rstride, out_tstride, pad);
    const int64_t nblocks = (int64_t)n_mtiles * nsplit * T;
    if (nblocks > 0x7fffffff) throw std::runtime_error("ppals: scan grid too large");
    const double bytes = (double)L * (double)J * (double)T * 4.0 + (double)L * (double)T * ncols * (out32 ? 4.0 : 8.0);
    prof_begin(0, bytes);
    dispatch<5, 6, 7, 8>(NT, [&](auto nt) {
      hipLaunchKernelGGL((k_scan_wide<nt, 1>), dim3((unsigned)nblocks), dim3(512), 0, st_, V, M, K, M * K, P,
                         n_mtiles, nsplit, per, nblk, d.p, d.nstride, d.split_stride, d.batch_stride, ncols, d.out32,
// ... 6 lines not shown
  }
  int gj_scalar_ = 0;
  bool wide_enabled_ = true;
  int wide_occ_[8] = {0, 0, 0, 0, 0, 0, 0, 0};
  template <typename TV>
  int scan_tail_split(int NT, int n_mtiles) {
    constexpr int VEC = ScanTraits<TV>::VEC;
    if (!scan_tail_on_) return -1;
    const size_t lds_t = sizeof(double) * 3 * (size_t)(VEC * NT * 4) * 64;
    const int per_cu = occupancy(scan_tail_occ_[(sizeof(TV) == 8 ? 2 : 0) + (NT - 1)],
                                 NT == 1 ? (const void *)k_scan_suffix_fast<TV, 1, 9>
                                         : (const void *)k_scan_suffix_fast<TV, 2, 9>,
                                 256, lds_t, -1);
    if (per_cu < 0) return -1;
    const int slots = ncu_ * per_cu;
    if (n_mtiles <= slots || n_mtiles > 4 * slots) return -1;
    const int rem = n_mtiles % slots;
    if (rem == 0 || rem * 4 > slots * 3) return -1;
    return n_mtiles - rem;
  }
  int scan_tail_occ_[4] = {0, 0, 0, 0};
  bool scan_tail_on_ = true;
  void scan_bf16(const uint16_t *V, int64_t L, int64_t J, int64_t T, const FactorRef *f, int nf, int R,
                 double *out, int64_t out_tstride, int64_t out_rstride, int out32, RowPad pad) {
    int64_t Jk;
    const KrpArgs a = krp_args(f, nf, &Jk);
    if (Jk != J) throw std::runtime_error("ppals: scan factor extents do not match the tensor");
    const bool aligned_base = (((uintptr_t)V) & 15) == 0;
    const int64_t nblk64 = (J + BF16_KB - 1) / BF16_KB;
    const int64_t n_mtiles64 = (L + 511) / 512;
    const bool mfma_ok = L > 1 && aligned_base && L % 8 == 0 && nblk64 * BF16_MAX_NT * 3 * 1024 < 2000000000ll &&
                         n_mtiles64 * T <= 0x7fffffff;
    const bool big = (double)BF16_KB * L * 2.0 >= 2.0e9;
    const double bytes_v = (double)L * J * T * 2.0;
    for (int col0 = 0; col0 < R; col0 += 16 * BF16_MAX_NT) {
      const int ncols = std::min(16 * BF16_MAX_NT, R - col0);
      double *o = out32 ? (double *)((float *)out + (int64_t)col0 * out_rstride) : out + (int64_t)col0 * out_rstride;
      prof_begin(0, bytes_v + (double)L * T * ncols * (out32 ? 4.0 : 8.0));
      if (mfma_ok) {
        const int NT = (ncols + 15) / 16;
        const int nblk = (int)nblk64;
        uint16_t *P = (uint16_t *)ensure(ws_pack_, ws_pack_sz_, (size_t)nblk * NT * 3 * 1024);
        hipLaunchKernelGGL(k_krp_pack_bf16, dim3(grid_for((int64_t)nblk * NT * 512, 256)), dim3(256), 0, st_, P,
                           nblk, NT, a, J, col0, ncols);
        HIP_CHECK(hipGetLastError());
        const int64_t M = L;
        int want = 1;
        if (T == 1 && n_mtiles64 < (int64_t)ncu_ * 8)
          want = (int)std::min<int64_t>(((int64_t)ncu_ * 8 + n_mtiles64 - 1) / n_mtiles64,
                                        std::max(1, nblk / 16));
        else if (T > 1 && n_mtiles64 * T < ncu_ && (double)M * T * ncols * nblk / 4 * 8.0 < 64e6)
          want = (int)std::min<int64_t>(((int64_t)ncu_ * 2 + n_mtiles64 * T - 1) / (n_mtiles64 * T),
                                        std::max(1, nblk / 4));
        const KSplit ks = k_split(nblk, want);
        const int nsplit = ks.nsplit, per = (int)ks.per;
        if (n_mtiles64 * nsplit * T > 0x7fffffff) throw std::runtime_error("ppals: scan grid too large");
        const PassDst d = pass_dst(nsplit, M, T, ncols, o, out32, out_rstride, out_tstride, pad);
        const dim3 grid((unsigned)(n_mtiles64 * nsplit * T));
        const bool nts = nt_store(nsplit, (double)L * T * ncols * (out32 ? 4.0 : 8.0));
        dispatch<true, false>(nts, [&](auto ntsv) {
          dispatch<true, false>(big, [&](auto bigv) {
            hipLaunchKernelGGL((k_scan_suffix_bf16<BF16_MAX_NT, ntsv, bigv>), grid, dim3(256), 0, st_, V, L, J, P,
                               (int)n_mtiles64, nsplit, per, nblk, d.p, d.nstride, d.split_stride, d.batch_stride,
                               ncols, d.out32, d.row_ld, d.row_valid);
          });
        });
        HIP_CHECK(hipGetLastError());
        slab_combine(nsplit, d.p, d.split_stride, M, ncols, o, 1, out_rstride, out32, pad, T, d.batch_stride,
                     out_tstride);
      } else {
        double *B = (double *)ensure(ws_krp_, ws_krp_sz_, sizeof(double) * (size_t)J * ncols);
        krp(B, f, nf, col0, ncols);
        if (L == 1)
          hipLaunchKernelGGL(k_scan_bf16_prefix<16 * BF16_MAX_NT>, dim3((unsigned)std::min<int64_t>((T + 3) / 4, 65536)),
                             dim3(256), 0,
                             st_, V, J, T, B, ncols, o, out_tstride, out_rstride, out32);
        else
          hipLaunchKernelGGL(k_scan_bf16_rows<16 * BF16_MAX_NT>, dim3(grid_for(L * T, 256, 16384)), dim3(256), 0,
                             st_, V, L, J, T, B, ncols, o, out_tstride, out_rstride, out32, pad.ld, pad.valid);
      }
      prof_end();
      HIP_CHECK(hipGetLastError());
    }
  }
  using Ops::scan_contract;
  void scan_contract(const void *V, int dt, int64_t L, int64_t J, int64_t T, const FactorRef *f,
                     int nf, int R, void *out, int out_dt, int64_t out_tstride,
                     int64_t out_rstride, RowPad pad) override {
    RoctxRange roctx_("K1/K2/K8/K11 tensor scan");
    const int out32 = out_dt == F32 ? 1 : 0;
    if (dt == BF16)
      scan_bf16((const uint16_t *)V, L, J, T, f, nf, R, (double *)out, out_tstride, out_rstride, out32,
                pad);
    else if (dt == F32)
      scan_t<float>((const float *)V, L, J, T, f, nf, R, (double *)out, out_tstride, out_rstride,
                    out32, pad);
    else
      scan_t<double>((const double *)V, L, J, T, f, nf, R, (double *)out, out_tstride,
                     out_rstride, out32, pad);
  }
  void ttm_keep(const void *X, int dt, int64_t L, int64_t J, int64_t T, const double *W, int64_t ldw,
                int Kc, double *out) override {
    const double bytes = (double)L * J * T * dtype_size(dt);
    if (L >= 16 && Kc <= 64 && bytes <= 64e6 && (double)L * J < 2e9 && T <= 65535 && J >= 16 &&
        (double)ldw * Kc < 4e9) {
      RoctxRange roctx_("K11 mode product (batched thin GEMM)");
      const int nt = Kc <= 16 ? 1 : (Kc <= 32 ? 2 : 4);
      dim3 grid((unsigned)((L + 15) / 16), (unsigned)((Kc + 16 * nt - 1) / (16 * nt)), (unsigned)T);
      prof_begin(1, bytes);
      dispatch<1, 2, 4>(nt, [&](auto ntv) {
        auto launch = [&](auto ta) {
          using TA = decltype(ta);
          hipLaunchKernelGGL((k_mode_product_small<TA, ntv>), grid, dim3(512), 0, st_, (const TA *)X, (int)L,
                             (int)J, W, ldw, Kc, out);
        };
        if (dt == F32) launch(float());
        else launch(double());
      });
      prof_end();
      HIP_CHECK(hipGetLastError());
      return;
    }
    Ops::ttm_keep(X, dt, L, J, T, W, ldw, Kc, out);
  }
  bool ttm_lead_front(const void *X, int dt, int64_t J, int64_t S, int64_t T, const double *W, int64_t ldw,
                      int Kc, double *out) override {
    const double bytes = (double)J * S * T * dtype_size(dt);
    if (!(S >= 16 && J >= 16 && Kc <= 64 && bytes <= 64e6 && (double)J * S < 2e9 && T <= 65535 &&
          (double)ldw * Kc < 4e9))
      return false;
    RoctxRange roctx_("K11 leading-mode product (batched thin GEMM)");
    const int nt = Kc <= 16 ? 1 : (Kc <= 32 ? 2 : 4);
    dim3 grid((unsigned)((S + 15) / 16), (unsigned)((Kc + 16 * nt - 1) / (16 * nt)), (unsigned)T);
    prof_begin(1, bytes);
    dispatch<1, 2, 4>(nt, [&](auto ntv) {
      auto launch = [&](auto ta) {
        using TA = decltype(ta);
        hipLaunchKernelGGL((k_mode_product_lead<TA, ntv>), grid, dim3(512), 0, st_, (const TA *)X, (int)J, (int)S,
                           W, ldw, Kc, out);
      };
      if (dt == F32) launch(float());
      else launch(double());
    });
    prof_end();
    HIP_CHECK(hipGetLastError());
    return true;
  }
  void pad_layout(const void *src, int dt, int64_t rows, int64_t cols, int64_t blk, int64_t ld,
                  void *dst) override {
    if (cols % blk || ld < blk) throw std::runtime_error("ppals: pad_layout block inconsistent");
    const size_t esz = dtype_size(dt);
    HIP_CHECK(hipMemsetAsync(dst, 0, (size_t)ld * (cols / blk) * rows * esz, st_));
    if (rows == 1) {
      HIP_CHECK(hipMemcpy2DAsync(dst, (size_t)ld * esz, src, (size_t)blk * esz, (size_t)blk * esz,
                                 (size_t)(cols / blk), hipMemcpyDeviceToDevice, st_));
      return;
    }
    const int64_t nb = ((rows + 63) / 64) * ((cols + 63) / 64);
    if (nb > 0x7fffffff) throw std::runtime_error("ppals: transpose grid too large");
    if (dt == F32)
      hipLaunchKernelGGL(k_transpose_pad<float>, dim3((unsigned)nb), dim3(256), 0, st_,
                         (const float *)src, rows, cols, blk, ld, (float *)dst);
    else if (dt == BF16)
      hipLaunchKernelGGL(k_transpose_pad<bf16s>, dim3((unsigned)nb), dim3(256), 0, st_,
                         (const bf16s *)src, rows, cols, blk, ld, (bf16s *)dst);
    else
// ... 1795 lines not shown
      throw std::runtime_error("ppals: rocSOLVER symbols missing");
    if (create(&rs_.handle) != 0 || set_stream(rs_.handle, st_) != 0)
      throw std::runtime_error("ppals: rocblas handle creation failed");
    return rs_;
  }
  RocSolver rs_;
  struct Timer {
    hipEvent_t a = nullptr, b = nullptr;
    bool busy = false, ended = false;
  };
  std::vector<Timer> timers_;
  struct Ev {
    hipEvent_t a, b;
    int slot;
    double bytes;
  };
  void prof_begin(int slot, double bytes) {
    cur_ = -1;
    if (profiling_ < 1 + slot) return;
    if (nev_ == events_.size()) {
      if (events_.size() >= 16384) return;
      Ev e;
      if (hipEventCreate(&e.a) != hipSuccess || hipEventCreate(&e.b) != hipSuccess) return;
      events_.push_back(e);
    }
    cur_ = (int)nev_++;
    events_[cur_].slot = slot;
    events_[cur_].bytes = bytes;
    hipEventRecord(events_[cur_].a, st_);
  }
  void prof_end() {
    if (cur_ >= 0) hipEventRecord(events_[cur_].b, st_);
    cur_ = -1;
  }
  void *ensure(void *&p, size_t &sz, size_t need) {
    if (need > sz) {
      if (p) {
        HIP_CHECK(hipStreamSynchronize(st_));
        HIP_CHECK(hipFree(p));
      }
      size_t n = need + need / 4 + 256;
      HIP_CHECK(hipMalloc(&p, n));
      sz = n;
    }
    return p;
  }
  double *small(int n) { return (double *)ensure(ws_small_, ws_small_sz_, sizeof(double) * n); }

  struct PassDst {
    double *p;
    int out32;
    int64_t nstride, split_stride, batch_stride, row_ld, row_valid;
  };
  PassDst pass_dst(int nsplit, int64_t M, int64_t T, int ncols, double *o, int out32, int64_t out_rstride,
                   int64_t out_tstride, RowPad pad) {
    if (nsplit == 1) return {o, out32, out_rstride, 0, out_tstride, pad.ld, pad.valid};
    double *slab = (double *)ensure(ws_slab_, ws_slab_sz_, sizeof(double) * nsplit * ncols * M * T);
    return {slab, 0, M, (int64_t)ncols * M * T, (int64_t)ncols * M, 0, 0};
  }
  void slab_combine(int nsplit, const double *slab, int64_t split_stride, int64_t M, int ncols, double *out,
                    int64_t out_mstride, int64_t out_rstride, int out32, RowPad pad = RowPad(), int64_t T = 1,
                    int64_t slab_bstride = 0, int64_t out_bstride = 0) {
    if (nsplit == 1) return;
    hipLaunchKernelGGL(k_slab_reduce, dim3(grid_for(M * ncols, 256), (unsigned)T), dim3(256), 0, st_, slab, nsplit,
                       split_stride, M, ncols, out, out_mstride, out_rstride, out32, pad.ld, pad.valid, slab_bstride,
                       out_bstride);
    HIP_CHECK(hipGetLastError());
  }
  static constexpr double kNtMinBytes = 192.0 * 1048576.0;
  bool nt_store(int nsplit, double result_bytes) const {
    return nsplit == 1 && (scan_nt_mode_ < 0 ? result_bytes >= kNtMinBytes : scan_nt_mode_ == 1);
  }
  static int occupancy(int &cached, const void *kernel, int block, size_t lds, int fallback) {
    if (cached == 0) {
      int nb = 0;
      const hipError_t e = hipOccupancyMaxActiveBlocksPerMultiprocessor(&nb, kernel, block, lds);
      if (e != hipSuccess) (void)hipGetLastError();
      cached = (e == hipSuccess && nb > 0) ? nb : fallback;
    }
    return cached;
  }

  int dev_ = 0, ncu_ = 256, force_jacobi_ = 0, persist_mult_ = 40;
  int eig_debug_ = 0;
  SysArgs sys_;
  int sys_R_ = 0;
  bool sys_armed_ = false, sys_ready_ = false;
  NormArgs norm_;
  int norm_mode_ = -1;
  const double *norm_G_ = nullptr;
  bool norm_armed_ = false;
  bool eig_frob_once_ = false;
  void *ws_jac_ = nullptr;
  size_t ws_jac_sz_ = 0;
  int sym_lds_min_ = 768;
  int eig_defer_ok_ = 1;
  bool handover_ok_ = true;
  unsigned long long *handover_ = nullptr;
  unsigned long long handover_seq_ = 0;
  int eig_defer_fail_ = 0;
  int eig_defer_count_ = 0;
  int eig_cold_ = 1;
  void *ws_cold_ = nullptr;
  size_t ws_cold_sz_ = 0;
  double eig_sigma_scale_ = 0;
  int force_eiginv_ = 0;
  int eig_fast_ = 1;
  std::map<int, EigState> eig_state_;
  int eig_next_base_ = 0;
  void *eig_host_ = nullptr;
  void *ws_eig_ = nullptr, *ws_orth_ = nullptr, *ws_pow_ = nullptr, *ws_part2_ = nullptr;
  size_t ws_eig_sz_ = 0, ws_orth_sz_ = 0, ws_pow_sz_ = 0, ws_part2_sz_ = 0;
  hipStream_t st_ = nullptr;
  hipStream_t st2_ = nullptr;
  void *ws_mttv_ = nullptr;
  void *ws_mv_ = nullptr;
  size_t ws_mv_sz_ = 0;
  size_t ws_mttv_sz_ = 0;
  void *ws_pack_ = nullptr, *ws_slab_ = nullptr, *ws_krp_ = nullptr, *ws_part_ = nullptr,
       *ws_small_ = nullptr, *ws_big_ = nullptr, *ws_big2_ = nullptr;
  size_t ws_pack_sz_ = 0, ws_slab_sz_ = 0, ws_krp_sz_ = 0, ws_part_sz_ = 0, ws_small_sz_ = 0,
         ws_big_sz_ = 0, ws_big2_sz_ = 0;
  int profiling_ = 0;
  std::vector<Ev> events_;
  size_t nev_ = 0;
  int cur_ = -1;
};

Ops *make_hip_ops(int device) { return new HipOps(device); }
void hip_preload_eigensolver() { (void)eig_libs(); }

}
```

### pairwise-perturbation_amd/csrc/kernels_scan.hip.h

```cpp
#pragma once
#include <hip/hip_runtime.h>
#include <stdint.h>

namespace ppals {

typedef float f32x4 __attribute__((ext_vector_type(4)));
typedef double f64x4 __attribute__((ext_vector_type(4)));
typedef double f64x2 __attribute__((ext_vector_type(2)));

template <typename TV>
struct ScanTraits;
template <>
struct ScanTraits<float> {
  static constexpr int VEC = 4;
  typedef f32x4 vec;
  typedef f32x4 acc;
  static constexpr bool NEEDS_FLUSH = true;
  __device__ static inline acc mfma(float a, float b, acc c) {
    return __builtin_amdgcn_mfma_f32_16x16x4f32(a, b, c, 0, 0, 0);
  }
  __device__ static inline int row(int lane, int reg) { return (lane >> 4) * 4 + reg; }
};
template <>
struct ScanTraits<double> {
// ... 369 lines not shown
      extern __shared__ double tail_lds[];
      constexpr int NS = VEC * NT * 4;
      if (wave > 0) {
#pragma unroll
        for (int a = 0; a < VEC; a++)
#pragma unroll
          for (int nt = 0; nt < NT; nt++)
#pragma unroll
            for (int r = 0; r < 4; r++) {
              double v;
              if constexpr (TR::NEEDS_FLUSH)
                v = acc64[a][nt][r];
              else
                v = (double)acc[a][nt][r];
              tail_lds[((wave - 1) * NS + (a * NT + nt) * 4 + r) * 64 + lane] = v;
            }
      }
      __syncthreads();
      if (wave > 0) return;
#pragma unroll
      for (int w = 0; w < 3; w++)
#pragma unroll
        for (int a = 0; a < VEC; a++)
#pragma unroll
          for (int nt = 0; nt < NT; nt++)
#pragma unroll
            for (int r = 0; r < 4; r++) {
              const double v = tail_lds[(w * NS + (a * NT + nt) * 4 + r) * 64 + lane];
              if constexpr (TR::NEEDS_FLUSH)
                acc64[a][nt][r] += v;
              else
                acc[a][nt][r] += v;
            }
    }
  }
  const int64_t obase = split * out_split_stride + batch * out_batch_stride;
  const ScanRowMap rm = scan_row_map<VEC>(m, M, row_ld, row_valid);
  const bool vec_ok =
      (((obase | out_nstride | rm.mo) & (VEC - 1)) == 0) && rm.nvalid == VEC;
#pragma unroll
  for (int nt = 0; nt < NT; nt++)
#pragma unroll
    for (int r = 0; r < 4; r++) {
      const int n = 16 * nt + TR::row(lane, r);
      if (n < ncols && rm.nvalid > 0) {
        double val[VEC];
#pragma unroll
        for (int jj = 0; jj < VEC; jj++) {
          if constexpr (TR::NEEDS_FLUSH)
            val[jj] = acc64[jj][nt][r];
          else
            val[jj] = (double)acc[jj][nt][r];
        }
        const int64_t idx = obase + (int64_t)n * out_nstride + rm.mo;
        if (vec_ok && out32) {
          typedef float ovec_t __attribute__((ext_vector_type(VEC)));
          ovec_t ov;
#pragma unroll
          for (int jj = 0; jj < VEC; jj++) ov[jj] = (float)val[jj];
          if constexpr (OPT & 4)
            __builtin_nontemporal_store(ov, reinterpret_cast<ovec_t *>(reinterpret_cast<float *>(out) + idx));
          else
            *reinterpret_cast<ovec_t *>(reinterpret_cast<float *>(out) + idx) = ov;
        } else if (vec_ok) {
#pragma unroll
          for (int jj = 0; jj < VEC; jj += 2) {
            f64x2 ov = {val[jj], val[jj + 1]};
            if constexpr (OPT & 4)
              __builtin_nontemporal_store(ov, reinterpret_cast<f64x2 *>(out + idx + jj));
            else
              *reinterpret_cast<f64x2 *>(out + idx + jj) = ov;
          }
        } else {
#pragma unroll
          for (int jj = 0; jj < VEC; jj++)
            if (jj < rm.nvalid) scan_store(out, idx + jj, val[jj], out32);
        }
      }
    }
}

typedef unsigned int scan_u32x4 __attribute__((vector_size(16)));

template <typename TV, int NT, int OPT = 1>
__global__ __launch_bounds__(256) void k_scan_suffix_buf(
    const TV *__restrict__ V, int64_t M, int64_t K, int64_t batch_stride,
    const TV *__restrict__ P, int n_mtiles, int nsplit, int kb_per_split, int nkb,
    double *__restrict__ out, int64_t out_nstride, int64_t out_split_stride,
    int64_t out_batch_stride, int ncols, int out32, int64_t ntiles, int64_t row_ld = 0,
    int64_t row_valid = 0) {
  typedef ScanTraits<TV> TR;
  typedef typename TR::vec vec;
  typedef typename TR::acc acc_t;
  constexpr int VEC = TR::VEC;
  constexpr int KB = 4 * VEC;
  constexpr int FLUSH = 4;
  constexpr int AUXV = (OPT & 1) ? 2 : 0;

  const int lane = threadIdx.x & 63, wave = threadIdx.x >> 6;
  const int g = lane >> 4, j16 = lane & 15;
  const int voffP = (int)((g * 16 + j16) * VEC * (int)sizeof(TV));
  const int64_t block_bytes = (int64_t)KB * M * (int64_t)sizeof(TV);
  const int64_t total_bytes = K * M * (int64_t)sizeof(TV);
  const int ustep = (int)((int64_t)4 * M * (int64_t)sizeof(TV));
  const __amdgpu_buffer_rsrc_t rsrcP = __builtin_amdgcn_make_buffer_rsrc(
      (void *)P, 0, (int)((int64_t)nkb * NT * (4 * 16 * VEC) * (int64_t)sizeof(TV)), 0x00020000);

  struct Tile {
    int64_t m, obase;
    const TV *vbase;
    int voff, kb0, kb1;
    bool live;
  };
  auto decode = [&](int64_t id, Tile &t) {
    unsigned b = (unsigned)id;
    const int mtile = (int)(b % (unsigned)n_mtiles);
    b /= (unsigned)n_mtiles;
    const int split = (int)(b % (unsigned)nsplit);
    const int64_t batch = b / (unsigned)nsplit;
    const int64_t m0 = ((int64_t)mtile * 4 + wave) * (16 * VEC);
    t.live = m0 < M;
    t.m = m0 + (int64_t)VEC * j16;
    const int64_t m_ld = t.live ? min(t.m, M - VEC) : 0;
    t.voff = (int)(((int64_t)g * M + m_ld) * (int64_t)sizeof(TV));
    t.kb0 = split * kb_per_split;
    t.kb1 = min(nkb, t.kb0 + kb_per_split);
    t.vbase = V + batch * batch_stride;
    t.obase = split * out_split_stride + batch * out_batch_stride;
  };
#define PPALS_BUF_LOAD(vbase_, voff_, kb_, vv_, bb_)                                           \
  {                                                                                            \
    const int64_t boff_ = (int64_t)(kb_)*block_bytes;                                          \
    const int64_t rem_ = total_bytes - boff_;                                                  \
    const __amdgpu_buffer_rsrc_t rs_ = __builtin_amdgcn_make_buffer_rsrc(                      \
        (void *)((const char *)(vbase_) + boff_), 0, (int)min(rem_, block_bytes), 0x00020000); \
    _Pragma("unroll") for (int u = 0; u < VEC; u++) vv_[u] = __builtin_bit_cast(               \
        vec, __builtin_amdgcn_raw_buffer_load_b128(rs_, voff_, u * ustep, AUXV));              \
    _Pragma("unroll") for (int nt = 0; nt < NT; nt++) bb_[nt] = __builtin_bit_cast(            \
        vec, __builtin_amdgcn_raw_buffer_load_b128(                                            \
                 rsrcP, voffP, (int)(((kb_)*NT + nt) * (4 * 16 * VEC) * (int)sizeof(TV)), 0)); \
  }

  Tile cur, nxt;
  int64_t id = blockIdx.x;
  for (; id < ntiles; id += gridDim.x) {
    decode(id, cur);
    if (cur.live && cur.kb0 < cur.kb1) break;
  }
  if (id >= ntiles) return;
  vec cv[VEC], cb[NT];
  PPALS_BUF_LOAD(cur.vbase, cur.voff, cur.kb0, cv, cb);

  for (;;) {
    bool has_next = false;
    int64_t nid = id + gridDim.x;
    for (; nid < ntiles; nid += gridDim.x) {
      decode(nid, nxt);
      if (nxt.live && nxt.kb0 < nxt.kb1) {
        has_next = true;
        break;
      }
    }
    acc_t acc[VEC][NT];
    double acc64[TR::NEEDS_FLUSH ? VEC : 1][TR::NEEDS_FLUSH ? NT : 1][4];
#pragma unroll
    for (int a = 0; a < VEC; a++)
#pragma unroll
      for (int nt = 0; nt < NT; nt++) {
#pragma unroll
        for (int r = 0; r < 4; r++) acc[a][nt][r] = 0;
        if constexpr (TR::NEEDS_FLUSH) {
#pragma unroll
          for (int r = 0; r < 4; r++) acc64[a][nt][r] = 0;
        }
      }
    for (int kc = cur.kb0; kc < cur.kb1; kc += FLUSH) {
      const int ke = min(cur.kb1, kc + FLUSH);
      for (int kb = kc; kb < ke; kb++) {
        vec nv[VEC], nb[NT];
        const bool same = kb + 1 < cur.kb1;
        const TV *pv = (same || !has_next) ? cur.vbase : nxt.vbase;
        const int po = (same || !has_next) ? cur.voff : nxt.voff;
        const int pk = same ? kb + 1 : (has_next ? nxt.kb0 : kb);
        PPALS_BUF_LOAD(pv, po, pk, nv, nb);
#pragma unroll
        for (int u = 0; u < VEC; u++)
#pragma unroll
          for (int jj = 0; jj < VEC; jj++)
#pragma unroll
            for (int nt = 0; nt < NT; nt++)
              acc[jj][nt] = TR::mfma(cb[nt][u], cv[u][jj], acc[jj][nt]);
#pragma unroll
        for (int u = 0; u < VEC; u++) cv[u] = nv[u];
#pragma unroll
        for (int nt = 0; nt < NT; nt++) cb[nt] = nb[nt];
      }
      if constexpr (TR::NEEDS_FLUSH) {
#pragma unroll
        for (int a = 0; a < VEC; a++)
#pragma unroll
          for (int nt = 0; nt < NT; nt++)
#pragma unroll
            for (int r = 0; r < 4; r++) {
              acc64[a][nt][r] += (double)acc[a][nt][r];
              acc[a][nt][r] = 0;
            }
      }
    }
    const ScanRowMap rm = scan_row_map<VEC>(cur.m, M, row_ld, row_valid);
    const bool vec_ok =
        (((cur.obase | out_nstride | rm.mo) & (VEC - 1)) == 0) && rm.nvalid == VEC;
#pragma unroll
    for (int nt = 0; nt < NT; nt++)
#pragma unroll
      for (int r = 0; r < 4; r++) {
        const int n = 16 * nt + TR::row(lane, r);
        if (n < ncols && rm.nvalid > 0) {
          double val[VEC];
#pragma unroll
          for (int jj = 0; jj < VEC; jj++) {
            if constexpr (TR::NEEDS_FLUSH)
              val[jj] = acc64[jj][nt][r];
            else
              val[jj] = (double)acc[jj][nt][r];
          }
          int64_t idx = cur.obase + (int64_t)n * out_nstride + rm.mo;
          if constexpr (OPT & 2)
            idx = cur.obase + (cur.m >> 8) * ((int64_t)ncols << 8) + ((int64_t)n << 8) + (cur.m & 255);
          if (vec_ok && out32) {
            typedef float ovec_t __attribute__((ext_vector_type(VEC)));
            ovec_t ov;
#pragma unroll
            for (int jj = 0; jj < VEC; jj++) ov[jj] = (float)val[jj];
            if constexpr (OPT & 4)
              __builtin_nontemporal_store(ov, reinterpret_cast<ovec_t *>(reinterpret_cast<float *>(out) + idx));
            else
              *reinterpret_cast<ovec_t *>(reinterpret_cast<float *>(out) + idx) = ov;
          } else if (vec_ok) {
#pragma unroll
            for (int jj = 0; jj < VEC; jj += 2) {
              f64x2 ov = {val[jj], val[jj + 1]};
              if constexpr (OPT & 4)
                __builtin_nontemporal_store(ov, reinterpret_cast<f64x2 *>(out + idx + jj));
              else
                *reinterpret_cast<f64x2 *>(out + idx + jj) = ov;
            }
          } else {
#pragma unroll
            for (int jj = 0; jj < VEC; jj++)
              if (jj < rm.nvalid) scan_store(out, idx + jj, val[jj], out32);
          }
        }
      }
    if (!has_next) break;
    cur = nxt;
    id = nid;
  }
#undef PPALS_BUF_LOAD
}

template <int NT, int OPT = 0>
__global__ __launch_bounds__(512) void k_scan_wide(
    const float *__restrict__ V, int64_t M, int64_t K, int64_t batch_stride,
    const float *__restrict__ P, int n_mtiles, int nsplit, int kb_per_split, int nkb,
    double *__restrict__ out, int64_t out_nstride, int64_t out_split_stride,
    int64_t out_batch_stride, int ncols, int out32, int64_t row_ld = 0, int64_t row_valid = 0) {
  constexpr int BM = 64, BK = 16;
  constexpr int PITCH = BM + 16;
  constexpr int NTA = (NT + 3) / 4;
  constexpr int VSZ = BK * PITCH, PSZ = 512 * 4;
  __shared__ __attribute__((aligned(16))) float Vs[2][2 * VSZ];
  __shared__ __attribute__((aligned(16))) float Ps[2][2 * PSZ];

  const int tid = threadIdx.x, lane = tid & 63;
  const int wave = __builtin_amdgcn_readfirstlane(tid >> 6);
  const int g = lane >> 4, j16 = lane & 15;
  const int wm = wave & 1, wn = wave >> 1;
  const int nt0 = NTA * wn, ntc = max(0, min(NTA, NT - nt0));

  unsigned b = blockIdx.x;
  const int mtile = (int)(b % (unsigned)n_mtiles);
  b /= (unsigned)n_mtiles;
  const int split = (int)(b % (unsigned)nsplit);
  const int64_t batch = b / (unsigned)nsplit;
  const int64_t m0 = (int64_t)mtile * BM;
  const int kb0 = split * kb_per_split;
  const int kb1 = min(nkb, kb0 + kb_per_split);
  const int nb = kb1 - kb0;
  if (nb <= 0) return;
  const int nstages = (nb + 1) >> 1;

  const int mq = tid & 15, kk = (tid >> 4) & 15, hv = wave >> 2;
  const int64_t m_ld = min(m0 + 4 * mq, M - 4);
  const char *__restrict__ vbase = (const char *)(V + batch * batch_stride);
  const int voffV = (int)(((int64_t)kk * M + m_ld) * 4);
  const int64_t block_bytes = (int64_t)BK * M * 4, total_bytes = K * M * 4;
  const int voffP = tid * 16;
  const int vdst = hv * VSZ + kk * PITCH + 4 * mq;
  const __amdgpu_buffer_rsrc_t rsrcP = __builtin_amdgcn_make_buffer_rsrc(
      (void *)P, 0, wave < NT ? (int)((int64_t)nkb * NT * 1024) : 0, 0x00020000);
  constexpr int AUXV = (OPT & 1) ? 2 : 0;

  f32x4 gv[2], gp[2][2];
#define PPALS_WIDE_LOAD(set_, st_)                                                                     \
  {                                                                                                    \
    _Pragma("unroll") for (int h_ = 0; h_ < 2; h_++) {                                                 \
      const int kb_ = kb0 + min(2 * (st_) + h_, nb - 1);                                               \
      gp[set_][h_] = __builtin_bit_cast(                                                               \
          f32x4, __builtin_amdgcn_raw_buffer_load_b128(rsrcP, voffP, kb_ * (NT * 1024), 0));           \
    }                                                                                                  \
    const int i_ = 2 * (st_) + hv;                   \
    const int64_t boff_ = (int64_t)(kb0 + min(i_, nb - 1)) * block_bytes;                              \
    const __amdgpu_buffer_rsrc_t rs_ = __builtin_amdgcn_make_buffer_rsrc(                              \
        (void *)(vbase + boff_), 0, i_ < nb ? (int)min(total_bytes - boff_, block_bytes) : 0,          \
        0x00020000);                                                                                   \
    gv[set_] = __builtin_bit_cast(f32x4, __builtin_amdgcn_raw_buffer_load_b128(rs_, voffV, 0, AUXV));  \
  }
#define PPALS_WIDE_STAGE(set_, buf_)                                                         \
  {                                                                                          \
    *reinterpret_cast<f32x4 *>(&Vs[buf_][vdst]) = gv[set_];                                  \
    _Pragma("unroll") for (int h_ = 0; h_ < 2; h_++)                                         \
        *reinterpret_cast<f32x4 *>(&Ps[buf_][h_ * PSZ + 4 * tid]) = gp[set_][h_];            \
  }

  f32x4 acc[2][NTA];
  double acc64[2][NTA][4];
#pragma unroll
  for (int ms = 0; ms < 2; ms++)
#pragma unroll
    for (int i = 0; i < NTA; i++)
#pragma unroll
      for (int r = 0; r < 4; r++) {
        acc[ms][i][r] = 0;
        acc64[ms][i][r] = 0;
      }

  PPALS_WIDE_LOAD(0, 0);
  PPALS_WIDE_LOAD(1, min(1, nstages - 1));
  PPALS_WIDE_STAGE(0, 0);
  __syncthreads();
  for (int j0 = 0; j0 < nstages; j0 += 2) {
// ... 533 lines not shown
```

### pairwise-perturbation_amd/csrc/kernels_small.hip.h

```cpp
#pragma once
#include <hip/hip_runtime.h>
#include <stdint.h>

#include "kernels_scan.hip.h"

namespace ppals {

typedef double f64x4 __attribute__((ext_vector_type(4)));


__host__ __device__ inline uint64_t splitmix64(uint64_t x) {
  x += 0x9E3779B97F4A7C15ull;
  x = (x ^ (x >> 30)) * 0xBF58476D1CE4E5B9ull;
  x = (x ^ (x >> 27)) * 0x94D049BB133111EBull;
  return x ^ (x >> 31);
}
__host__ __device__ inline double u01(uint64_t seed, uint64_t idx) {
  uint64_t h = splitmix64(splitmix64(seed) ^ idx);
  return (double)(h >> 11) * (1.0 / 9007199254740992.0);
}

__device__ inline double wave_sum(double v) {
#pragma unroll
  for (int off = 32; off > 0; off >>= 1) v += __shfl_down(v, off, 64);
// ... 252 lines not shown
    const int64_t j = e % J;
    const int c = (int)(e / J);
    double v = 1.0;
    int64_t rem = j;
    for (int f = 0; f < a.nf; f++) {
      const int64_t jf = rem % a.rows[f];
      rem /= a.rows[f];
      v *= a.ptr[f][jf + a.ld[f] * (col0 + c)];
    }
    out[e] = v;
  }
}

__device__ inline double mttv_scale(const double *scale) { return scale ? *scale : 1.0; }

__device__ inline void gram_system_wave(const double *__restrict__ Gall, int N, int mode, int R,
                                        double lambda, double *__restrict__ S,
                                        double *__restrict__ Sinv, int force_jacobi, double *lds);
struct SysArgs {
  const double *Gall = nullptr;
  int N = 0, mode = 0;
  double lambda = 0;
  double *S = nullptr, *Sinv = nullptr;
  int force_jacobi = 0;
};
#define PPALS_SYS_BLOCK(sys_, R_, nblk_)                                                        \
  int nblk_ = (int)gridDim.x;                                                                   \
  if ((sys_).Gall) {                                                                            \
    nblk_ -= 1;                                                                                 \
    if ((int)blockIdx.x == nblk_) {                                                             \
      extern __shared__ double sys_lds_[];                                                      \
      if (threadIdx.x < 64)                                                                     \
        gram_system_wave((sys_).Gall, (sys_).N, (sys_).mode, R_, (sys_).lambda, (sys_).S,       \
                         (sys_).Sinv, (sys_).force_jacobi, sys_lds_);                           \
      return;                                                                                   \
    }                                                                                           \
  }

template <typename TX>
__global__ __launch_bounds__(64) void k_mttv_vec(const TX *__restrict__ X, int64_t L, int64_t J,
                                                 int64_t T, int R, const double *__restrict__ B,
                                                 int64_t ldb, double *__restrict__ out, int64_t rs,
                                                 int accumulate, const double *__restrict__ scale,
                                                 SysArgs sys = SysArgs()) {
  PPALS_SYS_BLOCK(sys, R, nblk)
  constexpr int VL = 16 / sizeof(TX);
  typedef TX vecx __attribute__((ext_vector_type(VL)));
  const int lane = threadIdx.x;
  const int64_t ltiles = (L + 64 * VL - 1) / (64 * VL);
  const int64_t total = ltiles * T * R;
  const double sc = mttv_scale(scale);
  for (int64_t blk = blockIdx.x; blk < total; blk += nblk) {
    const int64_t lt = blk % ltiles;
    const int64_t t = (blk / ltiles) % T;
    const int r = (int)(blk / (ltiles * T));
    const int64_t l = lt * 64 * VL + (int64_t)lane * VL;
    if (l >= L) continue;
    const TX *x = X + l + L * J * (t + T * (int64_t)r);
    const double *b = B + ldb * r;
    double acc[VL];
#pragma unroll
    for (int e = 0; e < VL; e++) acc[e] = 0;
    int64_t j = 0;
    for (; j + 3 < J; j += 4) {
      vecx v0 = *reinterpret_cast<const vecx *>(x + L * j);
      vecx v1 = *reinterpret_cast<const vecx *>(x + L * (j + 1));
      vecx v2 = *reinterpret_cast<const vecx *>(x + L * (j + 2));
      vecx v3 = *reinterpret_cast<const vecx *>(x + L * (j + 3));
      const double b0 = b[j], b1 = b[j + 1], b2 = b[j + 2], b3 = b[j + 3];
#pragma unroll
      for (int e = 0; e < VL; e++)
        acc[e] += ((double)v0[e] * b0 + (double)v1[e] * b1) + ((double)v2[e] * b2 + (double)v3[e] * b3);
    }
    for (; j < J; j++) {
      vecx v0 = *reinterpret_cast<const vecx *>(x + L * j);
      const double b0 = b[j];
#pragma unroll
      for (int e = 0; e < VL; e++) acc[e] += (double)v0[e] * b0;
    }
    double *o = out + l + L * t + rs * r;
#pragma unroll
    for (int e = 0; e < VL; e++) o[e] = accumulate ? (o[e] + sc * acc[e]) : sc * acc[e];
  }
}

template <typename TX, int NW>
__global__ __launch_bounds__(64 * NW) void k_mttv_l(const TX *__restrict__ X, int64_t L, int64_t J,
                                                    int64_t T, int R, const double *__restrict__ B,
                                                    int64_t ldb, double *__restrict__ out,
                                                    int64_t rs, int accumulate,
                                                    const double *__restrict__ scale,
                                                    SysArgs sys = SysArgs(), int jsplit = 1,
                                                    int64_t jchunk = 0,
                                                    double *__restrict__ partial = nullptr) {
  PPALS_SYS_BLOCK(sys, R, nblk)
  __shared__ double part[NW][64];
  const int lane = threadIdx.x & 63, wave = threadIdx.x >> 6;
  const int64_t ltiles = (L + 63) / 64;
  const int64_t total = ltiles * T * R * jsplit;
  const double sc = mttv_scale(scale);
  for (int64_t blk0 = blockIdx.x; blk0 < total; blk0 += nblk) {
    const int split = (int)(blk0 % jsplit);
    const int64_t blk = blk0 / jsplit;
    const int64_t jbeg = jsplit > 1 ? split * jchunk : 0;
    const int64_t jend = jsplit > 1 ? min(J, jbeg + jchunk) : J;
    const int64_t lt = blk % ltiles;
    const int64_t t = (blk / ltiles) % T;
    const int r = (int)(blk / (ltiles * T));
    const int P = L < 64 ? 64 / (int)L : 1;
    const int lp = L < 64 ? lane / (int)L : 0;
    const int64_t l = L < 64 ? lane % (int)L : lt * 64 + lane;
    const TX *x = X + l + L * J * (t + T * (int64_t)r);
    const double *b = B + ldb * r;
    double s0 = 0, s1 = 0, s2 = 0, s3 = 0;
    if (l < L && lp < P) {
      const int64_t st = (int64_t)NW * P;
      int64_t j = jbeg + (int64_t)wave * P + lp;
      for (; j + 3 * st < jend; j += 4 * st) {
        s0 += (double)x[L * j] * b[j];
        s1 += (double)x[L * (j + st)] * b[j + st];
        s2 += (double)x[L * (j + 2 * st)] * b[j + 2 * st];
        s3 += (double)x[L * (j + 3 * st)] * b[j + 3 * st];
      }
      for (; j < jend; j += st) s0 += (double)x[L * j] * b[j];
    }
    part[wave][lane] = (s0 + s1) + (s2 + s3);
    __syncthreads();
    if (wave == 0 && l < L && lp == 0) {
      double s = 0;
#pragma unroll
      for (int w = 0; w < NW; w++)
        for (int q = 0; q < P; q++) s += part[w][lane + (int)L * q];
      if (jsplit > 1) {
        partial[(int64_t)split * (L * T * R) + l + L * (t + T * (int64_t)r)] = s;
      } else {
        s *= sc;
        double *o = out + l + L * t + rs * r;
        *o = accumulate ? (*o + s) : s;
      }
    }
    __syncthreads();
  }
}
__global__ __launch_bounds__(256) void k_mttv_combine(const double *__restrict__ partial, int jsplit,
                                                      int64_t LT, int R, double *__restrict__ out,
                                                      int64_t rs, int accumulate,
                                                      const double *__restrict__ scale) {
  const int64_t n = LT * R;
  const double sc = mttv_scale(scale);
  for (int64_t e = (int64_t)blockIdx.x * blockDim.x + threadIdx.x; e < n; e += (int64_t)gridDim.x * blockDim.x) {
    double s = 0;
    for (int q = 0; q < jsplit; q++) s += partial[(int64_t)q * n + e];
    s *= sc;
    double *o = out + (e % LT) + rs * (e / LT);
    *o = accumulate ? (*o + s) : s;
  }
}
template <typename TX>
__global__ __launch_bounds__(256) void k_mttv_s(const TX *__restrict__ X, int L, int64_t J, int64_t T,
                                                int R, const double *__restrict__ B, int64_t ldb,
                                                double *__restrict__ out, int64_t rs, int accumulate,
                                                const double *__restrict__ scale,
                                                SysArgs sys = SysArgs()) {
  PPALS_SYS_BLOCK(sys, R, nblk)
  const int lane = threadIdx.x & 63;
  const int64_t wid = ((int64_t)blockIdx.x * blockDim.x + threadIdx.x) >> 6;
// ... 1438 lines not shown
```

### pairwise-perturbation_amd/csrc/ops.h

```cpp
#pragma once
#include <cstddef>
#include <cstdint>

#include "bf16.h"
#include "device_view.h"
#include "preload_policy.h"

namespace ppals {

enum DType { F32 = 0, F64 = 1, BF16 = 3 };
inline size_t dtype_size(int dt) { return dt == F32 ? 4 : (dt == BF16 ? 2 : 8); }
inline int work_dt(int storage) { return storage == BF16 ? F32 : storage; }

struct RowPad {
  int64_t ld = 0, valid = 0;
};

constexpr int MAX_ORDER = 8;

struct FactorRef {
  const double *ptr;
  int64_t rows;
  int64_t ld;
};
// ... 7 lines not shown
};

struct ProfileSlot {
  int64_t launches = 0;
  double ms = 0;
  double bytes = 0;
};

class Ops {
 public:
  virtual ~Ops() {}
  virtual void *alloc(size_t bytes) = 0;
  virtual void free(void *p) = 0;
  virtual void h2d(void *dst, const void *src, size_t bytes) = 0;
  virtual void d2h(void *dst, const void *src, size_t bytes) = 0;
  virtual void d2d(void *dst, const void *src, size_t bytes) = 0;
  virtual void zero(void *p, size_t bytes) = 0;
  virtual void sync() = 0;
  virtual void *stream() { return nullptr; }
  virtual void bind() {}
  virtual bool supports_storage(int dt) { return dt == F32 || dt == F64; }

  virtual void fill_uniform(void *V, int dt, int64_t l0, int64_t g0, int64_t row0, int64_t rest,
                            uint64_t seed, double lo, double hi) = 0;
  virtual void fill_laplacian(void *V, int dt, int64_t l0, int64_t g0, int64_t row0, int64_t rest,
                              int ndigits, int s) = 0;
  virtual void add_uniform_noise(void *V, int dt, int64_t l0, int64_t g0, int64_t row0,
                                 int64_t rest, uint64_t seed, double lo, double hi,
                                 double alpha) = 0;
  virtual void uniform_sumsq(int64_t l0, int64_t g0, int64_t row0, int64_t rest, uint64_t seed,
                             double lo, double hi, double *out) = 0;
  virtual void fill_rank(void *V, int dt, int64_t M, int64_t K, const double *Q, const double *P,
                         int R) = 0;
  virtual void residual_sq(const void *V, int dt, int64_t M, int64_t K, const double *Q,
                           const double *P, int R, double *out) = 0;
  virtual void upload_shard(void *V, int dt, const double *host_full, int64_t l0, int64_t g0,
                            int64_t row0, int64_t rest) = 0;

  virtual void download_shard(const void *V, int dt, double *host_full, int64_t l0, int64_t g0,
                              int64_t row0, int64_t rest) = 0;

  virtual void transpose2d(const void *src, int dt, int64_t rows, int64_t cols, void *dst) = 0;
  virtual void transpose_batched(const void *src, int dt, int64_t rows, int64_t cols, int64_t batch,
                                 void *dst) {
    const size_t step = (size_t)rows * cols * dtype_size(dt);
    for (int64_t b = 0; b < batch; b++)
      transpose2d((const char *)src + b * step, dt, rows, cols, (char *)dst + b * step);
  }
  virtual void pad_layout(const void *src, int dt, int64_t rows, int64_t cols, int64_t blk,
                          int64_t ld, void *dst) = 0;
  virtual void unpack_shards(const void *stage, int dt, int64_t s0, int64_t rest, int64_t blk,
                             int P, int64_t chunk_bytes, void *full) = 0;
  virtual void *try_alloc(size_t bytes) { return alloc(bytes); }
  virtual void scan_store_mode(int mode) { (void)mode; }
  virtual size_t mem_available() { return (size_t)-1; }

  struct PtrInfo {
    bool is_device = false;
    int device = -1;
    uint64_t base = 0, size = 0;
  };
  virtual bool device_ptr_info(const void * , PtrInfo * , std::string * ) {
    throw Unsupported("ppals: this back end has no device views");
  }
  virtual void copy_view(const ViewPlan & , int , void * , int ,
                         void * , int , void * ) {
    throw Unsupported("ppals: this back end has no device views");
  }
  virtual void model_to_view(const ModelPlan & , const double * , const double * ,
                             int , bool , void * , int ,
                             const void * , int , void * ) {
    throw Unsupported("ppals: this back end has no device views");
  }

  virtual void krp(double *out, const FactorRef *f, int nf, int col0, int ncols) = 0;

  virtual void scan_contract(const void *V, int dt, int64_t L, int64_t J, int64_t T,
                             const FactorRef *f, int nf, int R, void *out, int out_dt,
                             int64_t out_tstride, int64_t out_rstride, RowPad pad) = 0;
  void scan_contract(const void *V, int dt, int64_t L, int64_t J, int64_t T, const FactorRef *f,
                     int nf, int R, void *out, int out_dt, int64_t out_tstride,
                     int64_t out_rstride) {
    scan_contract(V, dt, L, J, T, f, nf, R, out, out_dt, out_tstride, out_rstride, RowPad());
  }
  virtual void ttm_keep(const void *X, int dt, int64_t L, int64_t J, int64_t T, const double *W,
                        int64_t ldw, int Kc, double *out) {
    FactorRef f;
    f.ptr = W;
    f.rows = J;
    f.ld = ldw;
    scan_contract(X, dt, L, J, T, &f, 1, Kc, out, F64, L * Kc, L);
  }

  virtual bool ttm_lead_front(const void * , int , int64_t , int64_t , int64_t ,
                              const double * , int64_t , int , double * ) {
    return false;
  }

  virtual void mttv(const void *X, int xdt, int64_t L, int64_t J, int64_t T, const FactorRef *f,
                    int nf, int R, double *out, int64_t out_rstride, int accumulate,
                    const double *out_scale) = 0;
  virtual void pp_correct(const double *M0, int64_t rows, int R, const PPTerm *terms, int nterms,
                          double *M) {
    d2d(M, M0, sizeof(double) * rows * R);
    for (int t = 0; t < nterms; t++) {
      FactorRef f;
      f.ptr = terms[t].dW;
      f.rows = terms[t].ny;
      f.ld = terms[t].lddw;
      if (terms[t].keep_first)
        mttv(terms[t].T, F64, rows, terms[t].ny, 1, &f, 1, R, M, rows, 1, nullptr);
      else
        mttv(terms[t].T, F64, 1, terms[t].ny, rows, &f, 1, R, M, rows, 1, nullptr);
    }
  }
  virtual void scale_update(double *dst, const double *scales, unsigned mask, int set_one) = 0;
  virtual void scale_update_many(double *dst, const double *scales, const unsigned *masks,
                                 unsigned active, unsigned fresh) {
    for (int k = 0; k < 32; k++)
      if ((active >> k) & 1u) scale_update(dst + k, scales, masks[k], (fresh >> k) & 1u);
  }
  virtual void normalize_ms(double *const *W, const int64_t *rows, int N, int R, double *Gall,
                            double *ms_dst, const unsigned *masks, unsigned active, unsigned fresh,
                            double *wsq = nullptr) {
    normalize(W, rows, N, R, Gall);
    if (active) scale_update_many(ms_dst, normalize_scales(), masks, active, fresh);
    if (wsq)
      for (int i = 0; i < N; i++) sumsq(W[i], rows[i] * R, wsq + 2 * i);
  }
  virtual const double *normalize_scales() = 0;

  virtual void gram(const double *W, int64_t rows, int64_t ld, int R, double *G) = 0;
  virtual void gram_system(const double *Gall, int N, int mode, int R, double lambda, double *S,
                           double *Sinv) = 0;
  virtual void cp_update(const double *M, int64_t ldm, const double *Wold, int64_t ldw,
                         double *Wnew, int64_t ldn, double *grad, int64_t ldg, int64_t rows,
                         int R, const double *S, const double *Sinv, double *gradsq,
                         const double *Winit, int64_t ldi, double *dW, int64_t ldd,
                         double ratio) = 0;
  virtual void cp_mode_update(double *Gall, int N, int mode, int R, double lambda, const double *M,
                              int64_t ldm, double *W, int64_t ldw, double *grad, int64_t ldg,
                              int64_t rows, double *gradsq, const double *Winit, int64_t ldi,
                              double *dW, int64_t ldd, double ratio, double *S, double *Sinv,
                              double *dwsq = nullptr) {
    gram_system(Gall, N, mode, R, lambda, S, Sinv);
    cp_update(M, ldm, W, ldw, W, ldw, grad, ldg, rows, R, S, Sinv, gradsq, Winit, ldi, dW, ldd,
              ratio);
    gram(W, rows, ldw, R, Gall + (size_t)mode * R * R);
    if (dwsq && Winit) sumsq(dW, rows * R, dwsq);
  }
  virtual void cp_mode_update_blocked(double *Gall, int N, int mode, int R, double lambda,
                                      const double *Mblk, int64_t blk, int P, double *scratch,
                                      double *W, int64_t ldw, double *grad, int64_t ldg, int64_t rows,
                                      double *gradsq, const double *Winit, int64_t ldi, double *dW,
                                      int64_t ldd, double ratio, double *S, double *Sinv) {
    unpack_blocks(Mblk, rows, rows, R, blk, P, scratch);
    cp_mode_update(Gall, N, mode, R, lambda, scratch, rows, W, ldw, grad, ldg, rows, gradsq, Winit, ldi,
                   dW, ldd, ratio, S, Sinv);
  }
  virtual void arm_gram_system(const double * , int , int , int ,
                               double , double * , double * ) {}
  virtual bool arm_normalize(double *const * , const int64_t * , int , int ,
                             double * , int , double * ,
                             double *  = nullptr, const unsigned *  = nullptr,
                             unsigned  = 0, unsigned  = 0) {
    return false;
// ... 65 lines not shown
```

### pairwise-perturbation_amd/csrc/ppals_api.cpp

```cpp
#include <cstdio>
#include <cstring>
#include <memory>
#include <stdexcept>
#include <set>
#include <string>

#include "../../include/ppals.h"
#include "backend.h"
#include "preload_policy.h"
#include "engine.h"
#include "tucker.h"

using namespace ppals;

static thread_local std::string g_err;

struct ppals_ctx {
  Ops *ops = nullptr;
  Comm *comm = nullptr;
  SelfComm self;
  Comm &c() { return comm ? *comm : self; }
  std::set<ppals_cp *> cps;
  std::set<ppals_tucker *> tks;
  std::set<ppals_tensor *> tensors;
// ... 286 lines not shown
                          strides, stream);
  API_END(PPALS_ERR_HIP)
}
int ppals_tensor_export_device(ppals_tensor *t, void *dst, int dst_dtype, const int64_t *box_lo,
                               const int64_t *box_len, const int64_t *strides, void *stream) {
  API_BEGIN
  return copy_device_view(t, DV_EXPORT, dst, dst_dtype, box_lo, box_len, strides, stream);
  API_END(PPALS_ERR_HIP)
}

static inline uint64_t sm64(uint64_t x) {
  x += 0x9E3779B97F4A7C15ull;
  x = (x ^ (x >> 30)) * 0xBF58476D1CE4E5B9ull;
  x = (x ^ (x >> 27)) * 0x94D049BB133111EBull;
  return x ^ (x >> 31);
}
void ppals_fill_uniform_host(double *out, int64_t n, uint64_t seed, uint64_t offset, double lo,
                             double hi) {
  const uint64_t s = sm64(seed);
  for (int64_t i = 0; i < n; i++) {
    uint64_t h = sm64(s ^ (offset + (uint64_t)i));
    out[i] = lo + (hi - lo) * ((double)(h >> 11) * (1.0 / 9007199254740992.0));
  }
}

int ppals_cp_create(ppals_ctx *ctx, ppals_tensor *V, int R, ppals_cp **out) {
  if (!ctx || !V || !out) return fail(PPALS_ERR_ARG, "NULL argument");
  if (R <= 0) return fail(PPALS_ERR_ARG, "rank must be positive");
  API_BEGIN
  std::unique_ptr<ppals_cp> s(new ppals_cp);
  s->ctx = ctx;
  s->eng = new CpEngine(*ctx->ops, ctx->c(), V->d, R);
  ctx->cps.insert(s.get());
  *out = s.release();
  return PPALS_OK;
  API_END(PPALS_ERR_HIP)
}
void ppals_cp_destroy(ppals_cp *s) {
  if (!s) return;
  delete s->eng;
  if (s->ctx) s->ctx->cps.erase(s);
  delete s;
}
int ppals_cp_set_factors(ppals_cp *s, const double *Wflat, const double *gradWflat) {
  if (!s || !s->eng || !Wflat) return fail(PPALS_ERR_ARG, "NULL argument");
  API_BEGIN
  s->eng->set_factors(Wflat, gradWflat);
  return PPALS_OK;
  API_END(PPALS_ERR_HIP)
}
int ppals_cp_get_factors(ppals_cp *s, double *Wflat, double *gradWflat) {
  if (!s || !s->eng) return fail(PPALS_ERR_ARG, "NULL argument");
  API_BEGIN
  s->eng->get_factors(Wflat, gradWflat);
  return PPALS_OK;
  API_END(PPALS_ERR_HIP)
}
int ppals_cp_set_schedule(ppals_cp *s, int schedule) {
  if (!s || !s->eng) return fail(PPALS_ERR_ARG, "NULL session");
  if (schedule != PPALS_SCHEDULE_DT && schedule != PPALS_SCHEDULE_MSDT)
    return fail(PPALS_ERR_ARG, "schedule must be PPALS_SCHEDULE_DT or PPALS_SCHEDULE_MSDT");
  API_BEGIN
  s->eng->set_schedule(schedule);
  return PPALS_OK;
  API_END(PPALS_ERR_HIP)
}
int ppals_cp_get_schedule(const ppals_cp *s) { return s && s->eng ? s->eng->schedule() : PPALS_ERR_ARG; }
int ppals_cp_placement_report(const ppals_cp *s, char *buf, int cap) {
  if (!s || !s->eng || !buf || cap <= 0) return fail(PPALS_ERR_ARG, "NULL argument");
  API_BEGIN
  const std::string r = s->eng->placement_report();
  if ((int)r.size() + 1 > cap) return fail(PPALS_ERR_ARG, "buffer too small");
  std::memcpy(buf, r.c_str(), r.size() + 1);
  return PPALS_OK;
  API_END(PPALS_ERR_HIP)
}
int ppals_cp_pp_build_stats(ppals_cp *s, int mode, int64_t *builds, double *seconds) {
  if (!s || !s->eng) return fail(PPALS_ERR_ARG, "NULL argument");
  API_BEGIN
  s->eng->pp_build_stats(mode, builds, seconds);
  return PPALS_OK;
  API_END(PPALS_ERR_HIP)
}
int ppals_cp_sweeps_dt(ppals_cp *s, int n, double lambda) {
  if (!s || !s->eng) return fail(PPALS_ERR_ARG, "NULL argument");
  API_BEGIN
  for (int i = 0; i < n; i++) s->eng->sweep_dt(lambda);
  return PPALS_OK;
  API_END(PPALS_ERR_HIP)
}
int ppals_cp_gradnorm(ppals_cp *s, double *out) {
  if (!s || !s->eng || !out) return fail(PPALS_ERR_ARG, "NULL argument");
  API_BEGIN
  *out = s->eng->gradnorm();
  return PPALS_OK;
  API_END(PPALS_ERR_HIP)
}
int ppals_cp_residual(ppals_cp *s, double *out) {
  if (!s || !s->eng || !out) return fail(PPALS_ERR_ARG, "NULL argument");
  API_BEGIN
  *out = s->eng->residual();
  return PPALS_OK;
  API_END(PPALS_ERR_HIP)
}
static int check_model_view(ppals_ctx *ctx, const TensorDesc &d, const char *what, int kind, void *dst,
                            int dst_dtype, const int64_t *box_lo, const int64_t *box_len,
                            const int64_t *strides, ViewArgs *a) {
  if (!dst) return fail(PPALS_ERR_ARG, "NULL pointer");
  if (kind != PPALS_MODEL && kind != PPALS_RESIDUAL) {
    g_err = std::string(what) + "`what` must be PPALS_MODEL (0) or PPALS_RESIDUAL (1)";
    return PPALS_ERR_ARG;
  }
  return check_desc_view(ctx, d, what, DV_EXPORT, dst, dst_dtype, box_lo, box_len, strides, a);
}
int ppals_cp_export_model_device(ppals_cp *s, int what, void *dst, int dst_dtype, const int64_t *box_lo,
                                 const int64_t *box_len, const int64_t *strides, void *stream) {
  if (!s || !s->eng) return fail(PPALS_ERR_ARG, "NULL session");
  API_BEGIN
  ViewArgs a;
  const int rc = check_model_view(s->ctx, s->eng->tensor(), "ppals_cp_export_model_device: ", what, dst,
                                  dst_dtype, box_lo, box_len, strides, &a);
  if (rc != PPALS_OK) return rc;
  s->eng->export_model(a, dst, what == PPALS_RESIDUAL, stream);
  return PPALS_OK;
  API_END(PPALS_ERR_HIP)
}
int ppals_tucker_export_model_device(ppals_tucker *s, int what, void *dst, int dst_dtype,
                                     const int64_t *box_lo, const int64_t *box_len,
                                     const int64_t *strides, void *stream) {
  if (!s || !s->eng) return fail(PPALS_ERR_ARG, "NULL session");
  API_BEGIN
  ViewArgs a;
  const int rc = check_model_view(s->ctx, s->eng->tensor(), "ppals_tucker_export_model_device: ", what,
                                  dst, dst_dtype, box_lo, box_len, strides, &a);
  if (rc != PPALS_OK) return rc;
  s->eng->export_model(a, dst, what == PPALS_RESIDUAL, stream);
  return PPALS_OK;
  API_END(PPALS_ERR_HIP)
}
int ppals_tree_node(ppals_cp *s, const char *key, double *out, int64_t *n) {
  if (!s || !s->eng || !key) return fail(PPALS_ERR_ARG, "NULL argument");
  API_BEGIN
  int64_t c = s->eng->tree_node(key, out);
  if (c < 0) return fail(PPALS_ERR_ARG, "ppals_tree_node: not a node of the dimension tree");
  if (n) *n = c;
  return PPALS_OK;
  API_END(PPALS_ERR_HIP)
}
int ppals_mttkrp(ppals_cp *s, int mode, double *M) {
  if (!s || !s->eng || !M) return fail(PPALS_ERR_ARG, "NULL argument");
  if (mode < 0 || mode >= s->eng->order()) return fail(PPALS_ERR_ARG, "mode out of range");
  API_BEGIN
  s->eng->mttkrp(mode, M);
  return PPALS_OK;
  API_END(PPALS_ERR_HIP)
}
int ppals_pp_operator(ppals_cp *s, const char *contracted, double *out, int64_t *n) {
  if (!s || !s->eng || !contracted) return fail(PPALS_ERR_ARG, "NULL argument");
  API_BEGIN
  int64_t c = s->eng->pp_operator(contracted, out);
  if (c < 0) return fail(PPALS_ERR_ARG, "ppals_pp_operator: bad mode string");
  if (n) *n = c;
  return PPALS_OK;
  API_END(PPALS_ERR_HIP)
}
int ppals_cp_gram_system(ppals_cp *s, int mode, double lambda, double *S, double *Sinv) {
// ... 148 lines not shown
```

### pairwise-perturbation_amd/ppals/__init__.py

```python
import ctypes as C
import os
import weakref

import numpy as np

F32, F64 = 0, 1
F16, BF16 = 2, 3
_HERE = os.path.dirname(os.path.abspath(__file__))
_LIBPATH = os.environ.get("PPALS_LIB", os.path.join(os.path.dirname(_HERE), "lib", "libppals.so"))
_lib = None

c_dp = C.POINTER(C.c_double)


class PpalsError(RuntimeError):
    pass


class _Opts(C.Structure):
    _fields_ = [("tol", C.c_double), ("timelimit", C.c_double), ("maxiter", C.c_int),
                ("lambda_", C.c_double), ("resprint", C.c_int), ("bench", C.c_int),
                ("tol_init", C.c_double), ("ratio_step", C.c_double), ("csv_path", C.c_char_p),
                ("csv_append", C.c_int), ("verbose", C.c_int),
                ("update_percentage", C.c_double)]


EXPORTS = [
    "ppals_last_error", "ppals_version", "ppals_preload_eigensolver", "ppals_ctx_create",
    "ppals_ctx_destroy",
    "ppals_get_unique_id", "ppals_ctx_init_comm", "ppals_ctx_rank", "ppals_ctx_nranks",
    "ppals_ctx_sync", "ppals_profile_enable", "ppals_profile_read", "ppals_profile_reset",
    "ppals_tensor_create", "ppals_tensor_destroy", "ppals_tensor_local_rows",
    "ppals_tensor_fill_cp", "ppals_tensor_fill_uniform", "ppals_tensor_upload",
    "ppals_tensor_download", "ppals_tensor_import_device", "ppals_tensor_export_device",
    "ppals_tensor_check_device_view",
    "ppals_tensor_fill_laplacian", "ppals_tensor_fill_collinear", "ppals_collinear_factors",
    "ppals_tensor_norm", "ppals_fill_uniform_host", "ppals_tree_node", "ppals_mttkrp",
    "ppals_pp_operator", "ppals_cp_residual", "ppals_cp_gram_system", "ppals_cp_create",
    "ppals_cp_destroy", "ppals_cp_set_factors", "ppals_cp_get_factors", "ppals_cp_sweeps_dt",
    "ppals_cp_gradnorm", "ppals_cp_dt", "ppals_cp_pp", "ppals_cp_pp_partupdate",
    "ppals_cpd_als", "ppals_cpd_als_lr", "ppals_cp_set_schedule", "ppals_cp_get_schedule", "ppals_cp_placement_report", "ppals_cp_pp_build_stats",
    "ppals_tucker_create",
    "ppals_tucker_destroy", "ppals_tucker_set_factors", "ppals_tucker_get_factors",
    "ppals_tucker_set_core",
    "ppals_tucker_hosvd", "ppals_tucker_ttmc", "ppals_tucker_sweeps_dt", "ppals_tucker_dt",
    "ppals_tucker_pp", "ppals_cp_export_model_device", "ppals_tucker_export_model_device",
]
MODEL, RESIDUAL = 0, 1


def lib(path=None):
    global _lib
    if _lib is None:
        p = path or _LIBPATH
        if not os.path.exists(p):
            raise PpalsError(f"{p} not found: build it with `make -C pairwise-perturbation_amd` "
                             "(there is no pure-Python or CPU fallback)")
        _lib = C.CDLL(p)
        _lib.ppals_last_error.restype = C.c_char_p
        _lib.ppals_version.restype = C.c_char_p
        if __name__ == "ppals" and b"TEST INFRASTRUCTURE" in _lib.ppals_version():
            _lib = None
            raise PpalsError(f"{p} is the test stand-in, not the HIP engine (no CPU fallback)")
    return _lib


def _check(rc, allow_bool=False):
    if rc < 0:
        raise PpalsError(f"ppals error {rc}: {lib().ppals_last_error().decode()}")
    return rc


def _dp(a):
    return a.ctypes.data_as(c_dp)


def _torch():
    import torch
    return torch


def flat(Ws):
    return np.concatenate([np.asfortranarray(W, dtype=np.float64).ravel(order="F") for W in Ws])


def unflat(wflat, lens, ranks):
    out, p = [], 0
    for s, r in zip(lens, ranks):
        out.append(wflat[p:p + s * r].reshape((s, r), order="F").copy(order="F"))
        p += s * r
    return out


def fill_uniform_host(n, seed, offset=0, lo=0.0, hi=1.0):
    out = np.empty(int(n), dtype=np.float64)
    lib().ppals_fill_uniform_host(_dp(out), C.c_int64(int(n)), C.c_uint64(seed),
                                  C.c_uint64(offset), C.c_double(lo), C.c_double(hi))
    return out


def init_factors(lens, R, seed):
    return [fill_uniform_host(s * R, seed + i).reshape((s, R), order="F")
            for i, s in enumerate(lens)]


def collinear_factors(lens, R, col_min=0.5, col_max=0.9, seed=0):
    wf = np.empty(sum(int(s) * R for s in lens))
    arr = (C.c_int64 * len(lens))(*[int(x) for x in lens])
    _check(lib().ppals_collinear_factors(len(lens), arr, R, C.c_double(col_min),
                                         C.c_double(col_max), C.c_uint64(seed), _dp(wf)))
    return unflat(wf, lens, [R] * len(lens))


def preload_eigensolver():
    _check(lib().ppals_preload_eigensolver())


class Context:

    def __init__(self, device=0):
        self.device = device
        self._h = C.c_void_p()
        self._children = weakref.WeakSet()
        _check(lib().ppals_ctx_create(C.byref(self._h), device))
# ... 166 lines not shown
            lib().ppals_tensor_destroy(self._h)
            self._h = C.c_void_p()

    def __del__(self):
        try:
            self.close()
        except Exception:
            pass


def _opts(tol=0.0, timelimit=5e3, maxiter=0, lam=0.0, resprint=10, bench=0, tol_init=1e-2,
          ratio_step=1.0, csv=None, csv_append=0, verbose=0, update_percentage=1.0):
    return _Opts(tol, timelimit, maxiter, lam, resprint, bench, tol_init, ratio_step,
                 csv.encode() if csv else None, csv_append, verbose, update_percentage)


class _ModelExport:
    _export_fn = None

    def export_model_device(self, ptr, dtype, shape, strides, lo=None, residual=False, stream=0):
        blo, blen = Tensor._box(self, shape, lo)
        st = (C.c_int64 * len(self.lens))(*[int(x) for x in strides])
        _check(getattr(lib(), self._export_fn)(self._h, RESIDUAL if residual else MODEL,
                                               C.c_void_p(int(ptr)), int(dtype), blo, blen, st,
                                               C.c_void_p(int(stream or 0))))
        return self

    def export_model_torch(self, out, residual=False, lo=None, stream=None):
        torch = _torch()
        ptr, code, shape, strides = self.V._torch_view(out, (torch.float32, torch.float64))
        return self.export_model_device(ptr, code, shape, strides, lo, residual, Tensor._stream(stream))

    def model_to_torch(self, dtype=None, residual=False):
        torch = _torch()
        out = torch.zeros(self.lens, dtype=dtype or torch.float32, device=f"cuda:{self.ctx.device}")
        self.export_model_torch(out, residual=residual)
        return out


class CP(_ModelExport):
    _export_fn = "ppals_cp_export_model_device"

    def __init__(self, ctx, V, R):
        self.ctx, self.V, self.R = ctx, V, R
        self.lens = V.lens
        self._h = C.c_void_p()
        _check(lib().ppals_cp_create(ctx._h, V._h, R, C.byref(self._h)))
        ctx._children.add(self)

    def set_factors(self, Ws, gradWs=None):
        wf = flat(Ws)
        gf = flat(gradWs) if gradWs is not None else None
        _check(lib().ppals_cp_set_factors(self._h, _dp(wf), _dp(gf) if gf is not None else None))

    def get_factors(self, with_grad=False):
        n = sum(s * self.R for s in self.lens)
        wf = np.empty(n)
        gf = np.empty(n) if with_grad else None
        _check(lib().ppals_cp_get_factors(self._h, _dp(wf), _dp(gf) if with_grad else None))
        W = unflat(wf, self.lens, [self.R] * len(self.lens))
        if with_grad:
            return W, unflat(gf, self.lens, [self.R] * len(self.lens))
        return W

    def set_schedule(self, schedule):
        code = {"dt": 0, "msdt": 1}[schedule] if isinstance(schedule, str) else int(schedule)
        _check(lib().ppals_cp_set_schedule(self._h, code))

    @property
    def schedule(self):
        return {0: "dt", 1: "msdt"}[_check(lib().ppals_cp_get_schedule(self._h))]

    def placement_report(self):
        import json
        buf = C.create_string_buffer(8192)
        _check(lib().ppals_cp_placement_report(self._h, buf, 8192))
        return json.loads(buf.value.decode())

    def pp_build_stats(self, mode=0):
        n, sec = C.c_int64(0), C.c_double(0)
        _check(lib().ppals_cp_pp_build_stats(self._h, mode, C.byref(n), C.byref(sec)))
        return n.value, sec.value

    def sweeps_dt(self, n, lam=0.0):
        _check(lib().ppals_cp_sweeps_dt(self._h, n, C.c_double(lam)))

    def gradnorm(self):
        out = C.c_double(0)
        _check(lib().ppals_cp_gradnorm(self._h, C.byref(out)))
        return out.value

    def residual(self):
        out = C.c_double(0)
        _check(lib().ppals_cp_residual(self._h, C.byref(out)))
        return out.value

    def tree_node(self, key, shape=None):
        n = C.c_int64(0)
        _check(lib().ppals_tree_node(self._h, key.encode(), None, C.byref(n)))
        out = np.empty(n.value)
        _check(lib().ppals_tree_node(self._h, key.encode(), _dp(out), C.byref(n)))
        return out.reshape(shape, order="F") if shape else out

    def mttkrp(self, mode):
        M = np.empty(self.lens[mode] * self.R)
        _check(lib().ppals_mttkrp(self._h, mode, _dp(M)))
        return M.reshape((self.lens[mode], self.R), order="F")

    def pp_operator(self, contracted, shape=None):
        n = C.c_int64(0)
        _check(lib().ppals_pp_operator(self._h, contracted.encode(), None, C.byref(n)))
        out = np.empty(n.value)
        _check(lib().ppals_pp_operator(self._h, contracted.encode(), _dp(out), C.byref(n)))
        return out.reshape(shape, order="F") if shape else out

    def gram_system(self, mode, lam=0.0):
        S = np.empty(self.R * self.R)
        Si = np.empty(self.R * self.R)
        _check(lib().ppals_cp_gram_system(self._h, mode, C.c_double(lam), _dp(S), _dp(Si)))
        return S.reshape((self.R, self.R), order="F"), Si.reshape((self.R, self.R), order="F")

    def run_dt(self, **kw):
        o = _opts(**kw)
        it = C.c_int(0)
        rc = _check(lib().ppals_cp_dt(self._h, C.byref(o), C.byref(it)))
        return rc, it.value

    def run_pp(self, **kw):
        o = _opts(**kw)
        it = C.c_int(0)
        rc = _check(lib().ppals_cp_pp(self._h, C.byref(o), C.byref(it)))
        return rc, it.value

    def cpd_als(self, optimizer, **kw):
        o = _opts(**kw)
        it = C.c_int(0)
        sw = C.c_double(0)
        rc = _check(lib().ppals_cpd_als(self._h, int(optimizer), C.byref(o), C.byref(sw),
                                        C.byref(it)))
        return rc, sw.value, it.value

    def cpd_als_lr(self, optimizer, update_rank, randomsvd=0, **kw):
        o = _opts(**kw)
        it = C.c_int(0)
        sw = C.c_double(0)
        rc = _check(lib().ppals_cpd_als_lr(self._h, int(optimizer), int(update_rank), int(randomsvd),
                                           C.byref(o), C.byref(sw), C.byref(it)))
        return rc, sw.value, it.value

    def run_pp_partupdate(self, **kw):
        o = _opts(**kw)
        it = C.c_int(0)
        rc = _check(lib().ppals_cp_pp_partupdate(self._h, C.byref(o), C.byref(it)))
        return rc, it.value

    def close(self):
        if self._h:
            lib().ppals_cp_destroy(self._h)
            self._h = C.c_void_p()

    def __del__(self):
        try:
            self.close()
        except Exception:
            pass

# ... 95 lines not shown
```

Baseline: 567.1.

## Fuse first leaf contraction into tensor scan epilogue with alternate dimension tree

When a new multi-sweep step starts and the next mode to update is first in the order, the f32 tensor scan kernel gains an epilogue. It accumulates the first leaf's MTTKRP result in LDS per workgroup, writes per-workgroup slabs, and reduces them in a new kernel that can also run the armed Gram system solve. The engine builds an alternate dimension tree in which that leaf hangs directly off the root, so the leaf no longer needs a separate contraction of the first-level intermediate. The cost is extra LDS traffic and barriers inside a bandwidth-bound scan, plus a per-workgroup slab reduction. Leaf statistics are exposed through a new API call.

```diff
diff --git a/include/ppals.h b/include/ppals.h
--- a/include/ppals.h
+++ b/include/ppals.h
@@ -82,6 +82,7 @@
 int ppals_cp_get_schedule(const ppals_cp *s);
 int ppals_cp_placement_report(const ppals_cp *s, char *buf, int cap);
 int ppals_cp_pp_build_stats(ppals_cp *s, int mode, int64_t *builds, double *seconds);
+int ppals_cp_scan_leaf_stats(const ppals_cp *s, int64_t *steps, int64_t *taken);
 int ppals_cp_sweeps_dt(ppals_cp *s, int n, double lambda);
 int ppals_cp_gradnorm(ppals_cp *s, double *out);
 
diff --git a/pairwise-perturbation_amd/csrc/engine.cpp b/pairwise-perturbation_amd/csrc/engine.cpp
--- a/pairwise-perturbation_amd/csrc/engine.cpp
+++ b/pairwise-perturbation_amd/csrc/engine.cpp
@@ -238,6 +238,7 @@
   if (const char *e = std::getenv("PPALS_TEST_BLOCKED_UPDATE")) test_blocks_ = std::atoi(e);
   if (N_ < 3) schedule_ = 0;
   if (const char *e = std::getenv("PPALS_PLACE_TUNE")) ms_tune_enabled_ = std::atoi(e) != 0;
+  if (const char *e = std::getenv("PPALS_SCAN_LEAF")) ms_leaf_on_ = std::atoi(e) != 0;
   if (N_ >= 3) {
     ms_set_roots(ms_choose_roots());
     ms_scales_ = (double *)ops_.alloc(sizeof(double) * 32);
@@ -448,6 +449,7 @@
     if (p < best_p0) {
       plan.Lc *= ext(m);
       plan.kept.push_back(m);
+      plan.nfront++;
     } else if (p < best_p0 + k) {
       plan.J *= ext(m);
       plan.set.push_back(m);
@@ -818,6 +820,25 @@
   ms_leaf_.assign(N_ - k, -1);
   for (size_t q = 0; q < ms_nodes_.size(); q++)
     if (ms_nodes_[q].lo == ms_nodes_[q].hi) ms_leaf_[ms_nodes_[q].lo] = (int)q;
+  ms_leaf_alt_.clear();
+  ms_alt_ = false;
+  const int n = N_ - k;
+  if (ms_leaf_on_ && n >= 2 && 2 * ms_nodes_.size() + 1 <= 32) {
+    const size_t first = ms_nodes_.size();
+    for (int c = 0; c < 2; c++) {
+      MsNode nd;
+      nd.lo = c == 0 ? 0 : 1;
+      nd.hi = c == 0 ? 0 : n - 1;
+      nd.parent = -1;
+      nd.slo = c == 0 ? 1 : 0;
+      nd.shi = c == 0 ? n - 1 : 0;
+      ms_nodes_.push_back(nd);
+    }
+    ms_build_tree(1, n - 1, (int)first + 1);
+    ms_leaf_alt_.assign(n, -1);
+    for (size_t q = first; q < ms_nodes_.size(); q++)
+      if (ms_nodes_[q].lo == ms_nodes_[q].hi) ms_leaf_alt_[ms_nodes_[q].lo] = (int)q;
+  }
   if (ms_nodes_.size() + 1 > 32) throw std::runtime_error("ppals: tensor order too large");
   ms_X_.slot = 0;
   for (size_t q = 0; q < ms_nodes_.size(); q++) ms_nodes_[q].t.slot = (int)q + 1;
@@ -949,12 +970,13 @@
   }
 }
 
-void CpEngine::ms_start_step(int first) {
+void CpEngine::ms_start_step(int first, int next_update) {
   const int k = ms_k_;
   ms_root_ = first;
   ms_order_.clear();
   for (int q = k; q < N_; q++) ms_order_.push_back((first + q) % N_);
   for (auto &n : ms_nodes_) n.t.valid = false;
+  ms_alt_ = false;
   const size_t xbytes = ms_X_bytes(first, k);
   const size_t slack = ms_tune_enabled_ ? ms_X_slack() : 0;
   if (!ms_X_override_ && ms_X_cap_ < xbytes + slack) {
@@ -975,7 +997,7 @@
     ms_set_roots(1);
     int r = (first + k - 1) % N_, guard = 0;
     while (((ms_excl_ >> r) & 1u) && guard++ < N_) r = (r - 1 + N_) % N_;
-    ms_start_step(r);
+    ms_start_step(r, next_update);
     return;
   }
   const void *src = pl.lay->ptr;
@@ -991,12 +1013,30 @@
   ms_X_.contracted = mask;
   if ((size_t)L * T * R_ * dtype_size(ms_X_.dt) != xbytes)
     throw std::runtime_error("ppals: internal error (first-level intermediate size)");
+  std::vector<FactorRef> kept;
+  int leaf_pos = -1;
+  MsNode *leaf_node = nullptr;
+  if (ms_leaf_on_ && !ms_leaf_alt_.empty() && !dist_ && !ms_X_override_ && ms_order_.size() >= 2 &&
+      next_update == ms_order_[0]) {
+    for (size_t q = 0; q < pl.kept.size(); q++) {
+      kept.push_back(fref(pl.kept[q], W_.data()));
+      if (pl.kept[q] == ms_order_[0]) leaf_pos = (int)q;
+    }
+    leaf_node = &ms_nodes_[ms_leaf_alt_[0]];
+    ms_reserve(leaf_node->t, sizeof(double) * (size_t)ext(ms_order_[0]) * R_);
+  }
   auto launch_scan = [&](int blk, int64_t off, int nt) {
     ms_X_.buf = ms_X_override_ ? (char *)ms_X_override_
                                : (char *)(blk == 1 && ms_X_alt_ ? ms_X_alt_ : ms_X_base_) + off;
     ops_.scan_store_mode(nt);
-    ops_.scan_contract(src, V_.dtype, pl.L, J, T, f.data(), (int)f.size(), R_, ms_X_.buf, ms_X_.dt,
-                       L, L * T, pl.pad);
+    if (leaf_pos >= 0 &&
+        ops_.scan_contract_leaf(src, V_.dtype, pl.L, J, T, f.data(), (int)f.size(), R_, ms_X_.buf, ms_X_.dt,
+                                pl.pad, kept.data(), (int)kept.size(), pl.nfront, leaf_pos,
+                                (double *)leaf_node->t.buf, ext(ms_order_[0]), nullptr))
+      ms_alt_ = true;
+    else
+      ops_.scan_contract(src, V_.dtype, pl.L, J, T, f.data(), (int)f.size(), R_, ms_X_.buf, ms_X_.dt,
+                         L, L * T, pl.pad);
     ops_.scan_store_mode(-1);
   };
   PlaceExplore &ex = ms_place_[first];
@@ -1040,6 +1080,18 @@
   }
   ms_X_.pending = false;
   ms_X_.valid = true;
+  ms_steps_++;
+  if (ms_alt_) {
+    RTensor &t = leaf_node->t;
+    t.dt = F64;
+    t.modes.assign(1, ms_order_[0]);
+    t.contracted = 0;
+    for (int m = 0; m < N_; m++)
+      if (m != ms_order_[0]) t.contracted |= 1u << m;
+    t.pending = false;
+    t.valid = true;
+    ms_leaf_taken_++;
+  }
   if (const char *tr = std::getenv("PPALS_TRACE_STEPS")) {
     if (FILE *f = std::fopen(tr, "a")) {
       const int li = (int)(pl.lay - lay_.data());
@@ -1056,13 +1108,15 @@
   if (ms_root_ < 0 || ((i - ms_root_ + N_) % N_) < ms_k_) {
     const int first = ms_next_root(i, ms_k_, ms_excl_);
     if (first < 0) throw std::runtime_error("ppals: no root set without the excluded modes");
-    ms_start_step(first);
+    ops_.arm_gram_system(G_, N_, i, R_, lambda, S_, Sinv_);
+    ms_start_step(first, i);
+  } else {
+    ops_.arm_gram_system(G_, N_, i, R_, lambda, S_, Sinv_);
   }
   int pos = -1;
   for (size_t q = 0; q < ms_order_.size(); q++)
     if (ms_order_[q] == i) pos = (int)q;
-  const int leaf = ms_leaf_[pos];
-  ops_.arm_gram_system(G_, N_, i, R_, lambda, S_, Sinv_);
+  const int leaf = ms_leaf_map()[pos];
   ms_compute(leaf);
   ms_norm_fused_ = false;
   if (last_of_sweep && (!dist_ || (i != 0 && (int64_t)sizeof(double) * V_.glens[i] * R_ <= small_msg_bytes_))) {
@@ -1213,6 +1267,7 @@
     ms_order_.clear();
     for (int q = 1; q < N_; q++) ms_order_.push_back((left + q) % N_);
     for (auto &nd : ms_nodes_) nd.t.valid = false;
+    ms_alt_ = false;
   } else {
     ms_X_override_ = lr_cache_[left];
     ms_start_step(left);
diff --git a/pairwise-perturbation_amd/csrc/engine.h b/pairwise-perturbation_amd/csrc/engine.h
--- a/pairwise-perturbation_amd/csrc/engine.h
+++ b/pairwise-perturbation_amd/csrc/engine.h
@@ -89,6 +89,10 @@
       pp_build_timed_ = mode > 0;
     }
   }
+  void scan_leaf_stats(int64_t *steps, int64_t *taken) const {
+    if (steps) *steps = ms_steps_;
+    if (taken) *taken = ms_leaf_taken_;
+  }
   void get_factors(double *Wflat, double *gradWflat);
 
   void sweep_dt(double lambda);
@@ -154,7 +158,7 @@
     std::vector<RTensor> tmp;
   };
   void ms_build_tree(int lo, int hi, int parent);
-  void ms_start_step(int root);
+  void ms_start_step(int root, int next_update = -1);
   void ms_compute(int idx);
   void ms_reserve(RTensor &t, size_t bytes);
   void ms_contract(const RTensor &src, int mode, RTensor &dst, const double *in_scale);
@@ -228,6 +232,11 @@
 
   std::vector<int> ms_order_;
   std::vector<int> ms_leaf_;
+  std::vector<int> ms_leaf_alt_;
+  bool ms_alt_ = false;
+  bool ms_leaf_on_ = true;
+  int64_t ms_steps_ = 0, ms_leaf_taken_ = 0;
+  const std::vector<int> &ms_leaf_map() const { return ms_alt_ ? ms_leaf_alt_ : ms_leaf_; }
   double *ms_scales_ = nullptr;
   const double *ms_scale_of(const RTensor &t) const { return t.pending ? ms_scales_ + t.slot : nullptr; }
 
@@ -294,6 +303,7 @@
     int64_t L = 1, Lc = 1, J = 1, T = 1;
     RowPad pad;
     std::vector<int> set, kept;
+    int nfront = 0;
   };
   bool plan_scan(int first, int k, bool natural_only, ScanPlan &plan);
   void check_tensor_generation();
diff --git a/pairwise-perturbation_amd/csrc/hip_ops.hip b/pairwise-perturbation_amd/csrc/hip_ops.hip
--- a/pairwise-perturbation_amd/csrc/hip_ops.hip
+++ b/pairwise-perturbation_amd/csrc/hip_ops.hip
@@ -134,7 +134,7 @@
     if (const char *v = getenv("PPALS_SCAN_TAIL")) scan_tail_on_ = atoi(v) != 0;
     if (const char *v = getenv("PPALS_SCAN_WIDE")) wide_enabled_ = atoi(v) != 0;
     if (const char *v = getenv("PPALS_COLD_SUBSPACE_FROM")) cold_subspace_from_ = std::max(65, atoi(v));
-    if (const char *v = getenv("PPALS_PERSIST_MULT")) persist_mult_ = std::max(1, atoi(v));
+    if (const char *v = getenv("PPALS_PERSIST_MULT")) persist_mult_ = leaf_mult_ = std::max(1, atoi(v));
     HIP_CHECK(hipFuncSetAttribute((const void *)k_rmult_chol,
                                   hipFuncAttributeMaxDynamicSharedMemorySize, 152 * 1024));
     HIP_CHECK(hipFuncSetAttribute((const void *)k_jacobi_onesided,
@@ -163,6 +163,7 @@
     if (ws_pack_) hipFree(ws_pack_);
     if (ws_mv_) hipFree(ws_mv_);
     if (ws_slab_) hipFree(ws_slab_);
+    if (ws_leaf_) hipFree(ws_leaf_);
     if (ws_krp_) hipFree(ws_krp_);
     if (ws_part_) hipFree(ws_part_);
     if (ws_small_) hipFree(ws_small_);
@@ -742,9 +743,16 @@
     HIP_CHECK(hipGetLastError());
   }
 
+  struct LeafReq {
+    ScanLeafArgs a;
+    double *M = nullptr;
+    int64_t ldm = 0;
+    const double *scale = nullptr;
+  };
   template <typename TV>
   void scan_t(const TV *V, int64_t L, int64_t J, int64_t T, const FactorRef *f, int nf, int R,
-              double *out, int64_t out_tstride, int64_t out_rstride, int out32, RowPad pad) {
+              double *out, int64_t out_tstride, int64_t out_rstride, int out32, RowPad pad,
+              const LeafReq *leaf = nullptr) {
     constexpr int VEC = ScanTraits<TV>::VEC;
     int64_t Jc;
     KrpArgs a = krp_args(f, nf, &Jc);
@@ -845,6 +853,39 @@
         const bool takes_tail = !takes_buf && al && M >= VEC && T == 1 && nsplit == 1 && NT <= 2 &&
                                 d.row_ld == 0 && scan_tail_split<TV>(NT, n_mtiles) >= 0;
         if (takes_tail) nts = false;
+        if (leaf && !(sizeof(TV) == 4 && takes_buf && NT == 1 && nsplit == 1 && d.row_ld == 0 && col0 == 0))
+          throw std::logic_error("ppals: a leaf was accepted for a scan that cannot carry it");
+        if (leaf) {
+          ScanLeafArgs la = leaf->a;
+          const int sl = la.ext[la.leaf];
+          dim3 grid_l((unsigned)std::min<int64_t>(nblocks, (int64_t)ncu_ * leaf_mult_));
+          la.slab = (double *)ensure(ws_leaf_, ws_leaf_sz_, sizeof(double) * (size_t)grid_l.x * sl * ncols);
+          const size_t lds_l = scan_leaf_lds_bytes(sl, ncols);
+          if constexpr (sizeof(TV) == 4)
+            dispatch<21, 17>(nts ? 21 : 17, [&](auto opt) {
+              hipLaunchKernelGGL((k_scan_suffix_buf<float, 1, opt>), grid_l, dim3(256), lds_l, st_, V, M, K, M * K, P,
+                                 n_mtiles, nsplit, per, nblk, d.p, d.nstride, d.split_stride, d.batch_stride,
+                                 ncols, d.out32, nblocks, d.row_ld, d.row_valid, la);
+            });
+          prof_end();
+          HIP_CHECK(hipGetLastError());
+          SysArgs sys;
+          size_t lds_s = 0;
+          int extra = 0;
+          if (sys_armed_ && sys_R_ == R) {
+            sys = sys_;
+            extra = 1;
+            lds_s = sizeof(double) * (2 * (size_t)R * (R + 1) + 64) + sizeof(int) * 64;
+          }
+          hipLaunchKernelGGL(k_leaf_reduce, dim3((unsigned)((sl * ncols + 15) / 16 + extra)), dim3(1024), lds_s, st_,
+                             la.slab, (int)grid_l.x, sl * ncols, sl, leaf->M, leaf->ldm, leaf->scale, sys);
+          if (extra) {
+            sys_ready_ = true;
+            sys_armed_ = false;
+          }
+          HIP_CHECK(hipGetLastError());
+          return;
+        }
         if (takes_tail) {
           const int tail_from = scan_tail_split<TV>(NT, n_mtiles);
           const int64_t strips = ((M + 16 * VEC - 1) / (16 * VEC)) - (int64_t)tail_from * 4;
@@ -1017,6 +1058,51 @@
       prof_end();
       HIP_CHECK(hipGetLastError());
     }
+  }
+  template <typename TV>
+  bool leaf_scan_ok(const TV *V, int64_t L, int64_t J, int64_t T, int R, RowPad pad, const FactorRef *kept,
+                    int nkept, int nfront, int leaf) const {
+    constexpr int VEC = ScanTraits<TV>::VEC;
+    if (R > 16 || L <= 1 || pad.ld || nkept > SCAN_LEAF_MAX_MODES || nfront < 1 || nfront > nkept ||
+        leaf < 0 || leaf >= nkept || (leaf != 0 && leaf < nfront))
+      return false;
+    int64_t pl = 1, pt = 1;
+    for (int q = 0; q < nkept; q++) {
+      if (kept[q].rows <= 0 || kept[q].rows > 0x7fffffff) return false;
+      (q < nfront ? pl : pt) *= kept[q].rows;
+    }
+    if (pl != L || pt != T) return false;
+    if ((((uintptr_t)V) & 15) != 0 || L % 4 != 0 || kept[0].rows % 4 != 0) return false;
+    if (leaf == 0 && kept[0].rows < 16 * VEC) return false;
+    if (scan_leaf_lds_bytes((int)kept[leaf].rows, R) > 48 * 1024) return false;
+    const int64_t nblk = (J + 4 * VEC - 1) / (4 * VEC);
+    const int64_t n_mtiles = (L + 64 * VEC - 1) / (64 * VEC);
+    if (T == 1 && n_mtiles < (int64_t)ncu_ * 8 && nblk >= 64) return false;
+    if (T > 1 && n_mtiles * T < ncu_) return false;
+    if (n_mtiles * T > 0x7fffffff) return false;
+    return 16.0 * (double)L * sizeof(TV) < 2.0e9 && (double)nblk * 4 * 16 * VEC * sizeof(TV) < 2.0e9;
+  }
+  bool scan_contract_leaf(const void *V, int dt, int64_t L, int64_t J, int64_t T, const FactorRef *f, int nf,
+                          int R, void *out, int out_dt, RowPad pad, const FactorRef *kept, int nkept,
+                          int nfront, int leaf, double *M, int64_t ldm, const double *in_scale) override {
+    if (dt != F32 || out_dt != F32) return false;
+    if (!leaf_scan_ok((const float *)V, L, J, T, R, pad, kept, nkept, nfront, leaf)) return false;
+    RoctxRange roctx_("K1 tensor scan + first leaf");
+    LeafReq lr;
+    for (int q = 0; q < nkept; q++) {
+      lr.a.W[q] = kept[q].ptr;
+      lr.a.ld[q] = kept[q].ld;
+      lr.a.ext[q] = (int)kept[q].rows;
+    }
+    lr.a.nmodes = nkept;
+    lr.a.nrow = nfront;
+    lr.a.leaf = leaf;
+    lr.a.wpt = (int)std::max<int64_t>(1, std::min<int64_t>(4, kept[0].rows / 64));
+    lr.M = M;
+    lr.ldm = ldm;
+    lr.scale = in_scale;
+    scan_t<float>((const float *)V, L, J, T, f, nf, R, (double *)out, L, L * T, 1, pad, &lr);
+    return true;
   }
   using Ops::scan_contract;
   void scan_contract(const void *V, int dt, int64_t L, int64_t J, int64_t T, const FactorRef *f,
@@ -2978,6 +3064,7 @@
   }
 
   int dev_ = 0, ncu_ = 256, force_jacobi_ = 0, persist_mult_ = 40;
+  int leaf_mult_ = 8;
   int eig_debug_ = 0;
   SysArgs sys_;
   int sys_R_ = 0;
@@ -3015,6 +3102,8 @@
   size_t ws_mttv_sz_ = 0;
   void *ws_pack_ = nullptr, *ws_slab_ = nullptr, *ws_krp_ = nullptr, *ws_part_ = nullptr,
        *ws_small_ = nullptr, *ws_big_ = nullptr, *ws_big2_ = nullptr;
+  void *ws_leaf_ = nullptr;
+  size_t ws_leaf_sz_ = 0;
   size_t ws_pack_sz_ = 0, ws_slab_sz_ = 0, ws_krp_sz_ = 0, ws_part_sz_ = 0, ws_small_sz_ = 0,
          ws_big_sz_ = 0, ws_big2_sz_ = 0;
   int profiling_ = 0;
diff --git a/pairwise-perturbation_amd/csrc/kernels_scan.hip.h b/pairwise-perturbation_amd/csrc/kernels_scan.hip.h
--- a/pairwise-perturbation_amd/csrc/kernels_scan.hip.h
+++ b/pairwise-perturbation_amd/csrc/kernels_scan.hip.h
@@ -475,13 +475,32 @@
 
 typedef unsigned int scan_u32x4 __attribute__((vector_size(16)));
 
+constexpr int SCAN_LEAF_MAX_MODES = 8;
+struct ScanLeafArgs {
+  const double *W[SCAN_LEAF_MAX_MODES] = {nullptr};
+  int64_t ld[SCAN_LEAF_MAX_MODES] = {0};
+  int ext[SCAN_LEAF_MAX_MODES] = {0};
+  int nmodes = 0, nrow = 0, leaf = 0, wpt = 1;
+  double *slab = nullptr;
+};
+inline size_t scan_leaf_lds_bytes(int ext_leaf, int ncols) {
+  return sizeof(double) * ((size_t)ext_leaf * ncols + 128);
+}
+__device__ inline void scan_lds_barrier() {
+  __builtin_amdgcn_fence(__ATOMIC_RELEASE, "workgroup", "local");
+  __builtin_amdgcn_s_barrier();
+  __builtin_amdgcn_fence(__ATOMIC_ACQUIRE, "workgroup", "local");
+}
+
 template <typename TV, int NT, int OPT = 1>
 __global__ __launch_bounds__(256) void k_scan_suffix_buf(
     const TV *__restrict__ V, int64_t M, int64_t K, int64_t batch_stride,
     const TV *__restrict__ P, int n_mtiles, int nsplit, int kb_per_split, int nkb,
     double *__restrict__ out, int64_t out_nstride, int64_t out_split_stride,
     int64_t out_batch_stride, int ncols, int out32, int64_t ntiles, int64_t row_ld = 0,
-    int64_t row_valid = 0) {
+    int64_t row_valid = 0, ScanLeafArgs lf = ScanLeafArgs()) {
+  constexpr bool LEAF = (OPT & 16) != 0;
+  static_assert(!LEAF || NT == 1, "the leaf epilogue serves one n-tile");
   typedef ScanTraits<TV> TR;
   typedef typename TR::vec vec;
   typedef typename TR::acc acc_t;
@@ -502,7 +521,7 @@
   struct Tile {
     int64_t m, obase;
     const TV *vbase;
-    int voff, kb0, kb1;
+    int voff, kb0, kb1, bt;
     bool live;
   };
   auto decode = [&](int64_t id, Tile &t) {
@@ -518,6 +537,10 @@
     t.voff = (int)(((int64_t)g * M + m_ld) * (int64_t)sizeof(TV));
     t.kb0 = split * kb_per_split;
     t.kb1 = min(nkb, t.kb0 + kb_per_split);
+    if constexpr (LEAF) {
+      if (!t.live) t.kb1 = min(t.kb1, t.kb0 + 1);
+    }
+    t.bt = (int)batch;
     t.vbase = V + batch * batch_stride;
     t.obase = split * out_split_stride + batch * out_batch_stride;
   };
@@ -534,11 +557,18 @@
                  rsrcP, voffP, (int)(((kb_)*NT + nt) * (4 * 16 * VEC) * (int)sizeof(TV)), 0)); \
   }
 
+  extern __shared__ double leaf_lds[];
+  const int leaf_ext = LEAF ? lf.ext[lf.leaf] : 0;
+  int leaf_par = 0;
+  if constexpr (LEAF) {
+    for (int e = threadIdx.x; e < leaf_ext * ncols; e += 256) leaf_lds[e] = 0.0;
+    scan_lds_barrier();
+  }
   Tile cur, nxt;
   int64_t id = blockIdx.x;
   for (; id < ntiles; id += gridDim.x) {
     decode(id, cur);
-    if (cur.live && cur.kb0 < cur.kb1) break;
+    if (LEAF || (cur.live && cur.kb0 < cur.kb1)) break;
   }
   if (id >= ntiles) return;
   vec cv[VEC], cb[NT];
@@ -549,7 +579,7 @@
     int64_t nid = id + gridDim.x;
     for (; nid < ntiles; nid += gridDim.x) {
       decode(nid, nxt);
-      if (nxt.live && nxt.kb0 < nxt.kb1) {
+      if (LEAF || (nxt.live && nxt.kb0 < nxt.kb1)) {
         has_next = true;
         break;
       }
@@ -645,11 +675,89 @@
           }
         }
       }
+    if constexpr (LEAF) {
+      const bool mine = cur.live && rm.nvalid == VEC;
+      unsigned rest = mine ? (unsigned)cur.m : 0u;
+      const int i0 = (int)(rest % (unsigned)lf.ext[0]);
+      rest /= (unsigned)lf.ext[0];
+      int ncl[4];
+      double w[4];
+#pragma unroll
+      for (int r = 0; r < 4; r++) {
+        ncl[r] = min(TR::row(lane, r), ncols - 1);
+        w[r] = 1.0;
+      }
+      int tleaf = 0;
+      for (int q = 1; q < lf.nmodes; q++) {
+        if (q == lf.nrow) rest = (unsigned)cur.bt;
+        const int ix = (int)(rest % (unsigned)lf.ext[q]);
+        rest /= (unsigned)lf.ext[q];
+        if (q == lf.leaf) {
+          tleaf = ix;
+          continue;
+        }
+        const double *wq = lf.W[q] + ix;
+        const int64_t ldq = lf.ld[q];
+#pragma unroll
+        for (int r = 0; r < 4; r++) w[r] *= wq[ldq * ncl[r]];
+      }
+      auto xval = [&](int jj, int r) -> double {
+        if constexpr (TR::NEEDS_FLUSH)
+          return acc64[jj][0][r];
+        else
+          return (double)acc[jj][0][r];
+      };
+      if (lf.leaf == 0) {
+        for (int w0 = 0; w0 < 4; w0 += lf.wpt) {
+          if (mine && wave >= w0 && wave < w0 + lf.wpt) {
+#pragma unroll
+            for (int r = 0; r < 4; r++)
+              if (TR::row(lane, r) < ncols) {
+                double *a = leaf_lds + TR::row(lane, r) * leaf_ext + i0;
+#pragma unroll
+                for (int jj = 0; jj < VEC; jj++) a[jj] += xval(jj, r) * w[r];
+              }
+          }
+          scan_lds_barrier();
+        }
+      } else {
+        const double *w0p = lf.W[0] + i0;
+        const int64_t ld0 = lf.ld[0];
+        double sum[4];
+#pragma unroll
+        for (int r = 0; r < 4; r++) {
+          double a = 0.0;
+#pragma unroll
+          for (int jj = 0; jj < VEC; jj++) a += xval(jj, r) * w0p[ld0 * ncl[r] + jj];
+          sum[r] = mine ? a * w[r] : 0.0;
+        }
+#pragma unroll
+        for (int off = 1; off < 16; off <<= 1)
+#pragma unroll
+          for (int r = 0; r < 4; r++) sum[r] += __shfl_xor(sum[r], off);
+        double *stage = leaf_lds + leaf_ext * ncols + leaf_par * 64;
+        if (j16 == 0) {
+#pragma unroll
+          for (int r = 0; r < 4; r++) stage[wave * 16 + TR::row(lane, r)] = sum[r];
+        }
+        scan_lds_barrier();
+        if (wave == 0 && lane < ncols)
+          leaf_lds[lane * leaf_ext + tleaf] +=
+              ((stage[lane] + stage[16 + lane]) + stage[32 + lane]) + stage[48 + lane];
+        leaf_par ^= 1;
+      }
+    }
     if (!has_next) break;
     cur = nxt;
     id = nid;
   }
 #undef PPALS_BUF_LOAD
+  if constexpr (LEAF) {
+    scan_lds_barrier();
+    double *dst = lf.slab + (int64_t)blockIdx.x * leaf_ext * ncols;
+    for (int e = 2 * (int)threadIdx.x; e < leaf_ext * ncols; e += 512)
+      *reinterpret_cast<f64x2 *>(dst + e) = f64x2{leaf_lds[e], leaf_lds[e + 1]};
+  }
 }
 
 template <int NT, int OPT = 0>
diff --git a/pairwise-perturbation_amd/csrc/kernels_small.hip.h b/pairwise-perturbation_amd/csrc/kernels_small.hip.h
--- a/pairwise-perturbation_amd/csrc/kernels_small.hip.h
+++ b/pairwise-perturbation_amd/csrc/kernels_small.hip.h
@@ -358,6 +358,36 @@
 #pragma unroll
     for (int e = 0; e < VL; e++) o[e] = accumulate ? (o[e] + sc * acc[e]) : sc * acc[e];
   }
+}
+
+__global__ __launch_bounds__(1024) void k_leaf_reduce(const double *__restrict__ slab, int nwg, int n,
+                                                      int rows, double *__restrict__ out, int64_t ldo,
+                                                      const double *__restrict__ scale,
+                                                      SysArgs sys = SysArgs()) {
+  PPALS_SYS_BLOCK(sys, n / rows, nblk)
+  __shared__ double part[64][16];
+  const int el = threadIdx.x & 15, slice = threadIdx.x >> 4;
+  const int e = (int)blockIdx.x * 16 + el;
+  double s0 = 0, s1 = 0;
+  if (e < n) {
+    const double *p = slab + e;
+    int wg = slice;
+#pragma unroll 2
+    for (; wg + 64 < nwg; wg += 128) {
+      s0 += p[(int64_t)wg * n];
+      s1 += p[(int64_t)(wg + 64) * n];
+    }
+    if (wg < nwg) s0 += p[(int64_t)wg * n];
+  }
+  part[slice][el] = s0 + s1;
+  lds_barrier();
+  if (slice == 0 && e < n) {
+    double s = 0;
+#pragma unroll 8
+    for (int k = 0; k < 64; k++) s += part[k][el];
+    out[(e % rows) + ldo * (e / rows)] = mttv_scale(scale) * s;
+  }
+  (void)nblk;
 }
 
 template <typename TX, int NW>
diff --git a/pairwise-perturbation_amd/csrc/ops.h b/pairwise-perturbation_amd/csrc/ops.h
--- a/pairwise-perturbation_amd/csrc/ops.h
+++ b/pairwise-perturbation_amd/csrc/ops.h
@@ -113,6 +113,13 @@
                      int nf, int R, void *out, int out_dt, int64_t out_tstride,
                      int64_t out_rstride) {
     scan_contract(V, dt, L, J, T, f, nf, R, out, out_dt, out_tstride, out_rstride, RowPad());
+  }
+  virtual bool scan_contract_leaf(const void * , int , int64_t , int64_t , int64_t ,
+                                  const FactorRef * , int , int , void * ,
+                                  int , RowPad , const FactorRef * , int ,
+                                  int , int , double * , int64_t ,
+                                  const double * ) {
+    return false;
   }
   virtual void ttm_keep(const void *X, int dt, int64_t L, int64_t J, int64_t T, const double *W,
                         int64_t ldw, int Kc, double *out) {
diff --git a/pairwise-perturbation_amd/csrc/ppals_api.cpp b/pairwise-perturbation_amd/csrc/ppals_api.cpp
--- a/pairwise-perturbation_amd/csrc/ppals_api.cpp
+++ b/pairwise-perturbation_amd/csrc/ppals_api.cpp
@@ -392,6 +392,11 @@
   return PPALS_OK;
   API_END(PPALS_ERR_HIP)
 }
+int ppals_cp_scan_leaf_stats(const ppals_cp *s, int64_t *steps, int64_t *taken) {
+  if (!s || !s->eng) return fail(PPALS_ERR_ARG, "NULL argument");
+  s->eng->scan_leaf_stats(steps, taken);
+  return PPALS_OK;
+}
 int ppals_cp_sweeps_dt(ppals_cp *s, int n, double lambda) {
   if (!s || !s->eng) return fail(PPALS_ERR_ARG, "NULL argument");
   API_BEGIN
diff --git a/pairwise-perturbation_amd/ppals/__init__.py b/pairwise-perturbation_amd/ppals/__init__.py
--- a/pairwise-perturbation_amd/ppals/__init__.py
+++ b/pairwise-perturbation_amd/ppals/__init__.py
@@ -39,7 +39,7 @@
     "ppals_pp_operator", "ppals_cp_residual", "ppals_cp_gram_system", "ppals_cp_create",
     "ppals_cp_destroy", "ppals_cp_set_factors", "ppals_cp_get_factors", "ppals_cp_sweeps_dt",
     "ppals_cp_gradnorm", "ppals_cp_dt", "ppals_cp_pp", "ppals_cp_pp_partupdate",
-    "ppals_cpd_als", "ppals_cpd_als_lr", "ppals_cp_set_schedule", "ppals_cp_get_schedule", "ppals_cp_placement_report", "ppals_cp_pp_build_stats",
+    "ppals_cpd_als", "ppals_cpd_als_lr", "ppals_cp_set_schedule", "ppals_cp_get_schedule", "ppals_cp_placement_report", "ppals_cp_pp_build_stats", "ppals_cp_scan_leaf_stats",
     "ppals_tucker_create",
     "ppals_tucker_destroy", "ppals_tucker_set_factors", "ppals_tucker_get_factors",
     "ppals_tucker_set_core",
@@ -372,6 +372,11 @@
         _check(lib().ppals_cp_pp_build_stats(self._h, mode, C.byref(n), C.byref(sec)))
         return n.value, sec.value
 
+    def scan_leaf_stats(self):
+        n, k = C.c_int64(0), C.c_int64(0)
+        _check(lib().ppals_cp_scan_leaf_stats(self._h, C.byref(n), C.byref(k)))
+        return n.value, k.value
+
     def sweeps_dt(self, n, lam=0.0):
         _check(lib().ppals_cp_sweeps_dt(self._h, n, C.c_double(lam)))
 
```

After: 559.2. 1.4% lower.
